# Haian-Jin/TensoIR

Measured on AMD Instinct MI355X. Metric: primary+secondary rays/sec at 4096 rays x 512 samples, higher is better.
Workload: dtype f32 io and field; decoders split-bf16 x3 (hi/lo operands, 3 MFMA products), fp32 accumulate; indirect light (secondary-ray records): fp16 shadow taps + fp16 single-product decoder, fp32 accumulate

## Files before the change

include/tensoir_hip.h:

```cpp
#ifndef TENSOIR_HIP_H
#define TENSOIR_HIP_H

#include <stdint.h>

#ifdef __cplusplus
extern "C" {
#endif

#define TIR_VERSION 100

#define TIR_OK               0
#define TIR_ERR_ARG         -1001
#define TIR_ERR_UNSUPPORTED -1002
#define TIR_ERR_NO_DEVICE   -1003

typedef struct TirField {
    float aabb_min[3];
    float aabb_max[3];
    float inv_aabb[3];
    int32_t grid[3];
    float step_size;
    float distance_scale;
    float density_shift;
    float weight_thres;
// ... 18 lines not shown
    float occ_hi[3];
    int32_t tune_lds_lines;
    int32_t tune_xcd_order;
    const float* dense_sigma;
    int32_t dense_pitch;
} TirField;

typedef struct TirFieldHalf {
    const void* aplane[3];
    const void* aline[3];
} TirFieldHalf;

#define TIR_HALF_MAX_JOBS 8
typedef struct TirHalfJob { const float* src; void* dst; int64_t n; unsigned* absmax; } TirHalfJob;
typedef struct TirHalfJobs { TirHalfJob job[TIR_HALF_MAX_JOBS]; } TirHalfJobs;

typedef struct TirMlp {
    const float* packed;
    int32_t feat_dim;
    int32_t pe;
    int32_t hidden;
    int32_t out_dim;
    int32_t act;
    int32_t tune_grid;
} TirMlp;

typedef struct TirEnvSG {
    const float* sgs;
    const float* rot;
    int32_t n_sg;
    int32_t n_lights;
} TirEnvSG;

int  tir_version(void);
const char* tir_error_string(int code);
int  tir_device_check(void);

int tir_pack_plane(const float* src, float* dst, int32_t C, int32_t H, int32_t W, void* stream);
int tir_pack_occupancy(const float* vol, uint8_t* nbr, int32_t W, int32_t H, int32_t D, void* stream);
int tir_pack_basis(const float* w, float* dst, int32_t app_dim, int32_t n_in, void* stream);
int tir_light_mean(const float* light_line, float* mean, int32_t L, int32_t n, void* stream);
int64_t tir_mlp_packed_floats(int32_t feat_dim, int32_t pe, int32_t hidden, int32_t out_dim);
int tir_pack_mlp(const float* w0, const float* b0, const float* w1, const float* b1,
                 const float* w2, const float* b2, int32_t feat_dim, int32_t pe, int32_t hidden,
                 int32_t out_dim, float* packed, void* stream);

int tir_vm_density_fwd(const TirField* f, const float* xyz, float* feat, float* sigma,
                       int64_t n, void* stream);

int tir_occupancy_query(const TirField* f, const float* xyz, uint8_t* hit, int64_t n, void* stream);

int tir_dense_alpha(const TirField* f, const float* lin_x, const float* lin_y, const float* lin_z,
                    int32_t gx, int32_t gy, int32_t gz, float length, float* alpha, void* stream);
int tir_alpha_pool(const float* alpha, int32_t gx, int32_t gy, int32_t gz, float thres, float* vol,
                   int32_t* bbox, void* stream);
int tir_filter_rays(const TirField* f, const float* rays, int64_t n, int32_t n_samples, int32_t bbox_only,
                    uint8_t* mask, void* stream);

int tir_dense_sigma_build(const TirField* f, float* vol, int32_t pitch, void* stream);
int tir_dense_sigma_fwd(const TirField* f, const float* xyz, float* feat, float* sigma, int64_t n, void* stream);

int tir_density_grad_fwd(const TirField* f, const float* xyz, float* sigma, float* grad,
                         float* normal, int64_t n, const int32_t* n_dev, void* stream);
int tir_density_feat_grad_fwd(const TirField* f, const float* xyz, float* feat, float* grad, int64_t n, void* stream);

int tir_vm_app_fwd(const TirField* f, const float* xyz, const int32_t* light_idx,
                   const int32_t* idx_map, float* rad_feat, float* int_feat, int32_t out_stride,
                   int32_t idx_div, int64_t n, const int32_t* n_dev, void* stream);

int tir_vm_app_jitter_fwd(const TirField* f, const float* xyz, int64_t n, const int32_t* n_dev, float scale,
                          uint64_t seed, uint64_t offset, const int64_t* rng_state, float* xyz_out,
                          float* int_feat, int32_t out_stride, void* stream);

int tir_vm_app_primary_fwd(const TirField* f, const float* xyz, const int32_t* light_idx, const int32_t* idx_map,
                           float* rad_feat, float* int_feat, int32_t out_stride, int64_t n, const int32_t* n_dev,
                           float scale, uint64_t seed, uint64_t offset, const int64_t* rng_state, float* xyz_out,
                           float* int_feat_jit, void* stream);
int tir_vm_app_primary_x3_fwd(const TirField* f, const float* xyz, const int32_t* light_idx, const int32_t* idx_map,
                              float* rad_feat, float* int_feat, int32_t out_stride, int64_t n, const int32_t* n_dev,
                              float scale, uint64_t seed, uint64_t offset, const int64_t* rng_state, float* xyz_out,
                              float* int_feat_jit, void* stream);
int tir_vm_app_fwd_x3(const TirField* f, const float* xyz, const int32_t* light_idx,
                      const int32_t* idx_map, float* rad_feat, float* int_feat, int32_t out_stride,
                      int32_t idx_div, int64_t n, const int32_t* n_dev, void* stream);
int tir_vm_app_fwd_bf16x3(const TirField* f, const float* xyz, const int32_t* light_idx,
                          const int32_t* idx_map, float* rad_feat, float* int_feat, int32_t out_stride,
                          int32_t idx_div, int64_t n, const int32_t* n_dev, void* stream);
int tir_vm_app_fwd_valu(const TirField* f, const float* xyz, const int32_t* light_idx,
                        const int32_t* idx_map, float* rad_feat, float* int_feat, int32_t out_stride,
                        int32_t idx_div, int64_t n, const int32_t* n_dev, void* stream);

int tir_mlp_fwd(const TirMlp* m, const float* feat, int32_t feat_stride, const float* aux,
                const int32_t* aux_map, int32_t aux_mod, float* out, int64_t n, const int32_t* n_dev,
        void* stream);
int tir_mlp_fwd_bf16x3(const TirMlp* m, const float* feat, int32_t feat_stride, const float* aux,
                       const int32_t* aux_map, int32_t aux_mod, float* out, int64_t n, const int32_t* n_dev,
        void* stream);

int tir_pack_half(const float* const* srcs, void* const* dsts, const int64_t* counts, int32_t n_tables, void* stream);
int tir_pack_half_checked(const float* const* srcs, void* const* dsts, const int64_t* counts, int32_t n_tables, float* absmax,
                          void* stream);
int tir_vm_app_fwd_h16(const TirField* f, const TirFieldHalf* fh, const float* xyz, const int32_t* light_idx,
                       const int32_t* idx_map, float* rad_feat, int32_t out_stride, int32_t idx_div, int64_t n,
                       const int32_t* n_dev, void* stream);

int tir_indirect_fused_fwd(const TirField* f, const TirFieldHalf* fh, const TirMlp* m, const float* xyz,
                           const int32_t* light_idx, const int32_t* rec_map, int32_t idx_div, int32_t aux_mod,
                           const float* table, float* out, int64_t n, const int32_t* n_dev, void* stream);

int tir_indirect_fused_hp_fwd(const TirField* f, const TirMlp* m, const float* xyz, const int32_t* light_idx,
                              const int32_t* rec_map, int32_t idx_div, int32_t aux_mod, const float* table, float* out,
                              int64_t n, const int32_t* n_dev, void* stream);

int tir_mlp_fwd_multi_bf16x3(const TirMlp* const* mlps, const float* const* feats, int32_t feat_stride,
                             const float* const* auxs, const int32_t* const* aux_maps, float* const* outs,
                             int32_t n_jobs, int64_t n, const int32_t* n_dev, void* stream);

int tir_mlp_aux_table(const TirMlp* m, const float* aux, int64_t n_aux, float* table, void* stream);
int tir_mlp_fwd_auxtab_bf16x3(const TirMlp* m, const float* feat, int32_t feat_stride, const float* table,
                              const int32_t* aux_map, int32_t aux_mod, float* out, int64_t n, const int32_t* n_dev,
                              void* stream);
int tir_mlp_fwd_auxtab_f16(const TirMlp* m, const float* feat, int32_t feat_stride, const float* table,
                           const int32_t* aux_map, int32_t aux_mod, float* out, int64_t n, const int32_t* n_dev,
                           void* stream);
int tir_mlp_train_fwd_auxtab_bf16x3(const TirMlp* m, const float* feat, int32_t feat_stride, const float* table,
                                    const int32_t* aux_map, int32_t aux_mod, float* out, float* h1, float* h2, int64_t n,
                                    const int32_t* n_dev, void* stream);
int tir_mlp_fwd_multi_auxtab_bf16x3(const TirMlp* const* mlps, const float* const* feats, int32_t feat_stride,
                                    const float* const* auxs, const int32_t* const* aux_maps,
                                    const float* const* tables, float* const* outs, int32_t n_jobs, int64_t n,
                                    const int32_t* n_dev, void* stream);
int tir_mlp_train_fwd_multi_bf16x3(const TirMlp* const* mlps, const float* const* feats, int32_t feat_stride,
                                   const float* const* auxs, const int32_t* const* aux_maps, float* const* outs,
                                   float* const* h1s, float* const* h2s, int32_t n_jobs, int64_t n,
                                   const int32_t* n_dev, void* stream);
int tir_mlp_fwd_bf16(const TirMlp* m, const float* feat, int32_t feat_stride, const float* aux,
                     const int32_t* aux_map, int32_t aux_mod, float* out, int64_t n, const int32_t* n_dev,
        void* stream);
int tir_mlp_fwd_valu(const TirMlp* m, const float* feat, int32_t feat_stride, const float* aux,
                     const int32_t* aux_map, int32_t aux_mod, float* out, int64_t n, const int32_t* n_dev,
        void* stream);

int tir_march_primary_fwd(const TirField* f, const float* rays, const float* ray_jitter,
                          int32_t B, int32_t S, float t_stop, float* weight, float* acc,
                          float* depth, float* t_end, int32_t* app_count,
                          unsigned long long* stats, void* stream);

int tir_march_primary_fused_fwd(const TirField* f, const float* rays, const float* ray_jitter,
                                int32_t B, int32_t S, float t_stop, float* weight, float* acc,
                                float* depth, float* t_end, int32_t* app_count, unsigned long long* stats,
                                float* viewdirs, int32_t* zero_words, int32_t n_zero, int32_t* ticket,
                                int32_t* offsets, int32_t cap, int32_t* total, void* stream);

int tir_exclusive_scan(const int32_t* counts, int32_t* offsets, int32_t n, void* stream);
int tir_exclusive_scan_capped(const int32_t* counts, int32_t* offsets, int32_t n, int32_t cap,
                              int32_t* total, void* stream);

int tir_record_check(const int32_t* const* counters, const int64_t* caps, int32_t n, int64_t* state,
                     int64_t* host_out, void* stream);

int tir_compact_primary(const TirField* f, const float* rays, const float* ray_jitter,
                        const float* weight, const int32_t* offsets, int32_t B, int32_t S,
                        int32_t* rec_ray, int32_t* rec_k, float* rec_w, float* rec_xyz,
                        void* stream);

#define TIR_MAP_STRIDE 20
int tir_composite_primary(const float* rays, const int32_t* offsets, const float* rec_w,
                          const float* rgb, const float* brdf, const float* brdf_jit,
                          const float* pred_normal, const float* derived_normal,
                          const float* acc, const float* depth, int32_t B, int32_t white_bg,
                          int32_t is_relight, float fixed_fresnel, float* out_maps, void* stream);

int tir_composite_primary_fused(const float* rays, const int32_t* offsets, const float* rec_w,
                                const float* rgb, const float* brdf, const float* brdf_jit,
                                const float* pred_normal, const float* derived_normal,
                                const float* acc, const float* depth, int32_t B, int32_t white_bg,
                                int32_t is_relight, float fixed_fresnel, float* out_maps, int32_t* ticket,
                                float* smooth_out, int64_t* rng_state, int64_t rng_step, void* stream);


int tir_march_secondary_fwd(const TirField* f, const float* origins, const int32_t* org_map,
                            const float* dirs, const int32_t* dir_map, const uint8_t* active,
                            int64_t n_rays, int32_t n_dirs, int32_t n_sample, const float* z_vals,
                            float t_stop, float* vis, float* one_minus_acc,
                            int32_t* rec_counter, int64_t rec_cap, int32_t* rec_ray,
                            float* rec_w, float* rec_xyz, int32_t* ray_rec_off,
                            int32_t* ray_rec_cnt, unsigned long long* stats, void* stream);

int tir_march_secondary_ids_fwd(const TirField* f, const float* origins, const int32_t* org_map,
                                const float* dirs, const int32_t* dir_map, const uint8_t* active,
                                int64_t n_rays, int32_t n_dirs, int32_t n_sample, const float* z_vals,
                                float t_stop, float* vis, float* one_minus_acc,
                                int32_t* rec_counter, int64_t rec_cap, int32_t* rec_ray,
                                float* rec_w, float* rec_xyz, int32_t* ray_rec_off,
                                int32_t* ray_rec_cnt, unsigned long long* stats, const int32_t* ray_ids,
                                const int32_t* n_ids_dev, void* stream);

int tir_accumulate_records(const int32_t* ray_rec_off, const int32_t* ray_rec_cnt,
                           const float* rec_w, const float* rec_rgb, int64_t n_rays,
                           float* indirect, void* stream);

int tir_env_sg_fwd(const TirEnvSG* e, const float* dirs, int32_t D, float* out, void* stream);

int tir_env_pixel_fwd(const float* light_rgbs, int32_t H, int32_t W, const float* rot, const float* dirs,
                      int32_t n_lights, int64_t n_dirs, int32_t softplus, float* env, void* stream);
int tir_env_pixel_bwd(const float* light_rgbs, int32_t H, int32_t W, const float* rot, const float* dirs,
                      int32_t n_lights, int64_t n_dirs, const float* g_env, float* g_light, void* stream);

int tir_shade_setup(const float* maps, const float* rays, const float* dirs, int32_t M,
                    int32_t D, float acc_thres, float* surf, uint8_t* active, void* stream);

int tir_shade_setup_compact(const float* maps, const float* rays, const float* dirs, int32_t M,
                            int32_t D, float acc_thres, float* surf, uint8_t* active, int32_t* pair_ids,
                            int32_t* n_active, float* vis, int32_t* ray_rec_cnt, int32_t pair_order, void* stream);

int tir_shade_integrate(const float* maps, const float* rays, const float* dirs,
                        const int32_t* light_idx, const float* vis, const float* indirect,
                        const float* env, const float* weight_d, int32_t M, int32_t D,
                        int32_t n_lights, int32_t equal_area, int32_t use_srgb, float acc_thres,
                        float* out_rgb, void* stream);

int tir_shade_integrate_records(const float* maps, const float* rays, const float* dirs,
                                const int32_t* light_idx, const float* vis, const int32_t* ray_rec_off,
                                const int32_t* ray_rec_cnt, const float* rec_w, const float* rec_rgb,
                                const float* env, const float* weight_d, int32_t M, int32_t D,
                                int32_t n_lights, int32_t equal_area, int32_t use_srgb, float acc_thres,
                                float* out_rgb, int32_t* reset_counter, void* stream);

int tir_relight_importance(const float* normal, const float* albedo, const float* rough,
                           const float* fresnel, const float* rays_d, const float* light_dir,
                           const float* light_rgb, const float* light_pdf, const float* vis,
                           int32_t M, int32_t Ns, float* out_rgb, void* stream);

int tir_env_sample_setup(const float* row_cdf, const float* col_cdf, int32_t H, int32_t W, const float* env_dir,
                         const float* normal, int32_t M, int32_t Ns, uint64_t seed, uint64_t offset,
                         int32_t* cell, uint8_t* active, void* stream);
int tir_env_sample_setup_list(const float* row_cdf, const float* col_cdf, int32_t H, int32_t W, const float* env_dir,
                                int32_t dir_stride, const float* normal, int32_t M, int32_t Ns, uint64_t seed, uint64_t offset,
                                int32_t bins_r, int32_t bins_c, int32_t block_pairs, const int32_t* row_guide,
                                const uint16_t* col_guide, int32_t guide_rows, int32_t guide_cols, int32_t* cell,
                                float* vis, int32_t* pair_ids, int32_t* n_active, void* stream);
int tir_relight_importance_cells(const float* normal, const float* albedo, const float* rough,
                                 const float* fresnel, const float* rays_d, const int32_t* cell,
                                 const float* env_dir, const float* env_rgb, const float* env_pdf,
                                 const float* vis, int32_t M, int32_t Ns, float* out_rgb, void* stream);
int tir_relight_importance_cells_packed(const float* normal, const float* albedo, const float* rough,
                                        const float* fresnel, const float* rays_d, const int32_t* cell,
                                        const float* env_cell, const float* vis, int32_t M, int32_t Ns,
                                        float* out_rgb, void* stream);
int tir_env_lookup(const float* env_rgb, int32_t H, int32_t W, const float* dirs, int64_t n, float* out, void* stream);

int tir_surface_compact(const float* maps, const float* rays, int32_t B, float acc_thres, float* surf, float* normal,
                        float* albedo, float* rough, float* fresnel, float* rays_d, int32_t* slot, int32_t* n_hit,
                        void* stream);
int tir_env_sample_setup_list_n(const float* row_cdf, const float* col_cdf, int32_t H, int32_t W, const float* env_dir,
                                int32_t dir_stride, const float* normal, int32_t M, int32_t Ns, uint64_t seed, uint64_t offset,
                                int32_t bins_r, int32_t bins_c, int32_t block_pairs, const int32_t* row_guide,
                                const uint16_t* col_guide, int32_t guide_rows, int32_t guide_cols, int32_t* cell,
                                float* vis, int32_t* pair_ids, int32_t* n_active, const int32_t* m_dev, void* stream);
int tir_relight_importance_cells_packed_n(const float* normal, const float* albedo, const float* rough,
                                          const float* fresnel, const float* rays_d, const int32_t* cell,
                                          const float* env_cell, const float* vis, int32_t M, int32_t Ns,
                                          float* out_rgb, const int32_t* m_dev, void* stream);
int tir_env_compose(const float* env_rgb, int32_t H, int32_t W, const float* dirs, int32_t dir_stride, int64_t n,
                    const int32_t* slot, const float* fg_rgb, float* out, int32_t out_stride, void* stream);

int tir_ggx_specular(const float* normal, const float* v, const float* l, const float* rough,
                     const float* fresnel, int32_t M, int32_t D, float* spec, void* stream);

typedef struct TirFieldGrad {
    float* dplane[3];
    float* dline[3];
    float* aplane[3];
    float* aline[3];
    float* light_line;
    float* light_mean;
} TirFieldGrad;

int tir_march_primary_train_fwd(const TirField* f, const float* rays, const float* ray_jitter,
                                int32_t B, int32_t S, float t_stop, float* weight, float* sigma,
                                float* acc, float* depth, float* t_end, int32_t* app_count, void* stream);

int tir_composite_primary_bwd(const float* rays, const int32_t* offsets, const int32_t* rec_k,
                              const float* rec_w, const float* rgb, const float* brdf,
                              const float* brdf_jit, const float* pred_normal,
                              const float* derived_normal, const float* acc, const float* depth,
                              int32_t B, int32_t S, int32_t white_bg, int32_t is_relight,
                              float fixed_fresnel, const float* g_maps, float* g_rgb, float* g_brdf,
                              float* g_brdf_jit, float* g_pred, float* g_der, float* g_weight,
                              float* g_acc, float* g_depth, void* stream);

int tir_march_primary_bwd(const TirField* f, const TirFieldGrad* g, const float* rays,
                          const float* ray_jitter, int32_t B, int32_t S, const float* sigma,
                          const float* weight, const float* g_weight, const float* g_acc,
                          const float* g_depth, float* g_feature, void* stream);

int tir_density_grad_bwd(const TirField* f, const TirFieldGrad* g, const float* xyz,
                         const float* g_normal, int64_t n, void* stream);

int tir_vm_density_bwd(const TirField* f, const TirFieldGrad* g, const float* xyz, const float* g_feat, int64_t n,
                       void* stream);
int tir_density_feat_bwd(const TirField* f, const TirFieldGrad* g, const float* xyz, const float* g_feat,
                         float* g_xyz_out, int64_t n, void* stream);
int tir_density_feat_grad_bwd(const TirField* f, const TirFieldGrad* g, const float* xyz, const float* v,
                              float* g_xyz_out, int64_t n, void* stream);

int tir_vm_app_bwd(const TirField* f, const TirFieldGrad* g, const float* xyz,
                   const int32_t* light_idx, const int32_t* idx_map, const float* g_rad,
                   const float* g_int, int32_t stride, int64_t n, float* y_rad, float* y_int,
                   void* stream);

int tir_mlp_train_fwd(const TirMlp* m, const float* feat, int32_t feat_stride, const float* aux,
                      const int32_t* aux_map, int32_t aux_mod, float* out, float* h1, float* h2,
                      int64_t n, const int32_t* n_dev, void* stream);
int tir_mlp_train_fwd_bf16x3(const TirMlp* m, const float* feat, int32_t feat_stride, const float* aux,
                             const int32_t* aux_map, int32_t aux_mod, float* out, float* h1, float* h2,
                             int64_t n, const int32_t* n_dev, void* stream);
int tir_mlp_inputs(const TirMlp* m, const float* feat, int32_t feat_stride, const float* aux,
                   const int32_t* aux_map, int32_t aux_mod, float* x, int64_t n, void* stream);
int64_t tir_mlp_bwd_packed_floats(int32_t feat_dim, int32_t pe, int32_t hidden, int32_t out_dim);
int tir_pack_mlp_bwd(const float* w0, const float* w1, const float* w2, int32_t feat_dim, int32_t pe,
                     int32_t hidden, int32_t out_dim, float* packed, void* stream);
int tir_mlp_bwd(const TirMlp* m, const float* packed_bwd, const float* feat, int32_t feat_stride,
                const float* out, const float* g_out, const float* h1, const float* h2, int64_t n,
                float* g_feat, float* dz1, float* dz2, float* dz3, void* stream);
int tir_mlp_bwd_bf16x3(const TirMlp* m, const float* packed_bwd, const float* feat, int32_t feat_stride,
                const float* out, const float* g_out, const float* h1, const float* h2, int64_t n,
                float* g_feat, float* dz1, float* dz2, float* dz3, void* stream);
int tir_mlp_bwd_multi_bf16x3(const TirMlp* const* mlps, const float* const* packed_bwds, const float* const* feats,
                             int32_t feat_stride, const float* const* outs, const float* const* g_outs,
                             const float* const* h1s, const float* const* h2s, int32_t n_jobs, int64_t n,
                             float* const* g_feats, float* const* dz1s, float* const* dz2s, float* const* dz3s, void* stream);

int tir_gemm_tn_small_bf16x3(const float* const* As, int32_t lda, int32_t M, const float* const* Bs, int32_t ldb,
                             int32_t N, int32_t n_jobs, int64_t n, float* C, int32_t ldc, void* stream);

int tir_mlp_wgrad_multi(const float* const* dz1s, const float* const* dz2s, const float* const* dz3s,
                        const float* const* h1s, const float* const* h2s, const float* const* feats,
                        int32_t feat_stride, const float* const* auxs, const int32_t* const* aux_maps,
                        float* const* dW0s, float* const* db0s, float* const* dW1s, float* const* db1s,
                        float* const* dW2s, float* const* db2s, int32_t n_jobs, int64_t n, int32_t max_workgroups,
                        void* stream);

int tir_gemm_tn(const float* A, int32_t lda, int32_t M, const float* B, int32_t ldb, int32_t N,
                int32_t ones_col, int64_t n, float* C, int32_t ldc, float* bias_out, void* stream);
int tir_gemm_tn_bf16x3(const float* A, int32_t lda, int32_t M, const float* B, int32_t ldb, int32_t N,
                int32_t ones_col, int64_t n, float* C, int32_t ldc, float* bias_out, void* stream);

int tir_adam_step(int32_t n_tensors, float* const* p, const float* const* g, float* const* m, float* const* v,
                  const int64_t* count, const float* lr, const float* bias_correction1,
                  const float* bias_correction2, float beta1, float beta2, float eps, void* stream);

int tir_shade_integrate_bwd(const float* maps, const float* rays, const float* dirs,
                            const int32_t* light_idx, const float* vis, const float* indirect,
                            const float* env, const float* weight_d, int32_t M, int32_t D,
                            int32_t n_lights, int32_t equal_area, int32_t use_srgb, float acc_thres,
                            const float* g_out, float* g_maps, float* g_env, void* stream);

int tir_env_sg_bwd(const TirEnvSG* e, const float* dirs, int32_t D, const float* g_env, float* g_sgs,
                   void* stream);

int64_t tir_mc_blocks(int32_t gx, int32_t gy, int32_t gz);
int tir_mc_count(const float* vol, int32_t gx, int32_t gy, int32_t gz, float level, int32_t* counts, int32_t* offsets,
                 void* stream);
int tir_mc_emit(const float* vol, int32_t gx, int32_t gy, int32_t gz, float level, float spacing_x, float spacing_y,
                float spacing_z, float origin_x, float origin_y, float origin_z, const int32_t* offsets, int32_t n_verts,
                int32_t n_faces, int32_t* vbase, float* verts, float* normals, int32_t* faces, void* stream);
// ... 100 lines not shown
```

tensoir_amd/_lib.py:

```python
from __future__ import annotations

import ctypes as C
import os

_HERE = os.path.dirname(os.path.abspath(__file__))
LIB_PATH = os.environ.get("TENSOIR_HIP_LIB", os.path.join(_HERE, "libtensoir_hip.so"))

c_float_p = C.c_void_p
c_int_p = C.c_void_p


class TirField(C.Structure):
    _fields_ = [
        ("aabb_min", C.c_float * 3), ("aabb_max", C.c_float * 3), ("inv_aabb", C.c_float * 3),
        ("grid", C.c_int32 * 3),
        ("step_size", C.c_float), ("distance_scale", C.c_float), ("density_shift", C.c_float),
        ("weight_thres", C.c_float), ("near_", C.c_float), ("far_", C.c_float),
        ("act", C.c_int32), ("n_dcomp", C.c_int32), ("n_acomp", C.c_int32), ("app_dim", C.c_int32),
        ("n_lights", C.c_int32),
        ("dplane", C.c_void_p * 3), ("dline", C.c_void_p * 3),
        ("aplane", C.c_void_p * 3), ("aline", C.c_void_p * 3),
        ("basis_t", C.c_void_p), ("light_line", C.c_void_p), ("light_mean", C.c_void_p),
        ("occ_nbr", C.c_void_p),
        ("occ_dim", C.c_int32 * 3), ("occ_aabb_min", C.c_float * 3), ("occ_inv", C.c_float * 3),
        ("occ_lo", C.c_float * 3), ("occ_hi", C.c_float * 3),
        ("tune_lds_lines", C.c_int32), ("tune_xcd_order", C.c_int32),
        ("dense_sigma", C.c_void_p), ("dense_pitch", C.c_int32),
    ]


class TirFieldHalf(C.Structure):
    _fields_ = [("aplane", C.c_void_p * 3), ("aline", C.c_void_p * 3)]


class TirFieldGrad(C.Structure):
    _fields_ = [("dplane", C.c_void_p * 3), ("dline", C.c_void_p * 3), ("aplane", C.c_void_p * 3),
                ("aline", C.c_void_p * 3), ("light_line", C.c_void_p), ("light_mean", C.c_void_p)]


class TirMlp(C.Structure):
    _fields_ = [("packed", C.c_void_p), ("feat_dim", C.c_int32), ("pe", C.c_int32),
                ("hidden", C.c_int32), ("out_dim", C.c_int32), ("act", C.c_int32), ("tune_grid", C.c_int32)]


class TirEnvSG(C.Structure):
    _fields_ = [("sgs", C.c_void_p), ("rot", C.c_void_p), ("n_sg", C.c_int32), ("n_lights", C.c_int32)]


P = C.c_void_p
I32 = C.c_int32
I64 = C.c_int64
F32 = C.c_float

SIGNATURES = {
    "tir_version": (C.c_int, []),
    "tir_error_string": (C.c_char_p, [C.c_int]),
    "tir_device_check": (C.c_int, []),
    "tir_pack_plane": (C.c_int, [P, P, I32, I32, I32, P]),
    "tir_pack_occupancy": (C.c_int, [P, P, I32, I32, I32, P]),
    "tir_pack_basis": (C.c_int, [P, P, I32, I32, P]),
    "tir_light_mean": (C.c_int, [P, P, I32, I32, P]),
    "tir_mlp_packed_floats": (I64, [I32, I32, I32, I32]),
    "tir_pack_mlp": (C.c_int, [P, P, P, P, P, P, I32, I32, I32, I32, P, P]),
    "tir_vm_density_fwd": (C.c_int, [C.POINTER(TirField), P, P, P, I64, P]),
    "tir_occupancy_query": (C.c_int, [C.POINTER(TirField), P, P, I64, P]),
    "tir_dense_alpha": (C.c_int, [C.POINTER(TirField), P, P, P, I32, I32, I32, F32, P, P]),
    "tir_alpha_pool": (C.c_int, [P, I32, I32, I32, F32, P, P, P]),
    "tir_filter_rays": (C.c_int, [C.POINTER(TirField), P, I64, I32, I32, P, P]),
    "tir_dense_sigma_build": (C.c_int, [C.POINTER(TirField), P, I32, P]),
    "tir_dense_sigma_fwd": (C.c_int, [C.POINTER(TirField), P, P, P, I64, P]),
    "tir_density_grad_fwd": (C.c_int, [C.POINTER(TirField), P, P, P, P, I64, P, P]),
    "tir_density_feat_grad_fwd": (C.c_int, [C.POINTER(TirField), P, P, P, I64, P]),
    "tir_vm_app_fwd": (C.c_int, [C.POINTER(TirField), P, P, P, P, P, I32, I32, I64, P, P]),
    "tir_vm_app_fwd_bf16x3": (C.c_int, [C.POINTER(TirField), P, P, P, P, P, I32, I32, I64, P, P]),
    "tir_vm_app_fwd_x3": (C.c_int, [C.POINTER(TirField), P, P, P, P, P, I32, I32, I64, P, P]),
    "tir_pack_half": (C.c_int, [P, P, P, I32, P]),
    "tir_pack_half_checked": (C.c_int, [P, P, P, I32, P, P]),
    "tir_vm_app_fwd_h16": (C.c_int, [C.POINTER(TirField), C.POINTER(TirFieldHalf), P, P, P, P, I32, I32, I64, P, P]),
    "tir_indirect_fused_fwd": (C.c_int, [C.POINTER(TirField), C.POINTER(TirFieldHalf), C.POINTER(TirMlp), P, P, P, I32, I32, P, P, I64, P, P]),
    "tir_indirect_fused_hp_fwd": (C.c_int, [C.POINTER(TirField), C.POINTER(TirMlp), P, P, P, I32, I32, P, P, I64, P, P]),
    "tir_vm_app_fwd_valu": (C.c_int, [C.POINTER(TirField), P, P, P, P, P, I32, I32, I64, P, P]),
    "tir_mlp_fwd": (C.c_int, [C.POINTER(TirMlp), P, I32, P, P, I32, P, I64, P, P]),
    "tir_mlp_fwd_bf16x3": (C.c_int, [C.POINTER(TirMlp), P, I32, P, P, I32, P, I64, P, P]),
    "tir_mlp_fwd_multi_bf16x3": (C.c_int, [P, P, I32, P, P, P, I32, I64, P, P]),
    "tir_mlp_fwd_multi_auxtab_bf16x3": (C.c_int, [P, P, I32, P, P, P, P, I32, I64, P, P]),
    "tir_mlp_aux_table": (C.c_int, [C.POINTER(TirMlp), P, I64, P, P]),
    "tir_mlp_fwd_auxtab_bf16x3": (C.c_int, [C.POINTER(TirMlp), P, I32, P, P, I32, P, I64, P, P]),
    "tir_mlp_fwd_auxtab_f16": (C.c_int, [C.POINTER(TirMlp), P, I32, P, P, I32, P, I64, P, P]),
    "tir_mlp_train_fwd_auxtab_bf16x3": (C.c_int, [C.POINTER(TirMlp), P, I32, P, P, I32, P, P, P, I64, P, P]),
    "tir_mlp_train_fwd_multi_bf16x3": (C.c_int, [P, P, I32, P, P, P, P, P, I32, I64, P, P]),
    "tir_mlp_fwd_bf16": (C.c_int, [C.POINTER(TirMlp), P, I32, P, P, I32, P, I64, P, P]),
    "tir_mlp_fwd_valu": (C.c_int, [C.POINTER(TirMlp), P, I32, P, P, I32, P, I64, P, P]),
    "tir_march_primary_fwd": (C.c_int, [C.POINTER(TirField), P, P, I32, I32, F32, P, P, P, P, P, P, P]),
    "tir_exclusive_scan": (C.c_int, [P, P, I32, P]),
    "tir_exclusive_scan_capped": (C.c_int, [P, P, I32, I32, P, P]),
    "tir_march_primary_fused_fwd": (C.c_int, [C.POINTER(TirField), P, P, I32, I32, F32, P, P, P, P, P, P,
                                              P, P, I32, P, P, I32, P, P]),
    "tir_composite_primary_fused": (C.c_int, [P, P, P, P, P, P, P, P, P, P, I32, I32, I32, F32, P, P, P, P, I64, P]),
    "tir_vm_app_jitter_fwd": (C.c_int, [C.POINTER(TirField), P, I64, P, F32, C.c_uint64, C.c_uint64, P, P, P, I32, P]),
    "tir_vm_app_primary_fwd": (C.c_int, [C.POINTER(TirField), P, P, P, P, P, I32, I64, P, F32, C.c_uint64, C.c_uint64, P, P, P, P]),
    "tir_vm_app_primary_x3_fwd": (C.c_int, [C.POINTER(TirField), P, P, P, P, P, I32, I64, P, F32, C.c_uint64, C.c_uint64, P, P, P, P]),
    "tir_compact_primary": (C.c_int, [C.POINTER(TirField), P, P, P, P, I32, I32, P, P, P, P, P]),
    "tir_composite_primary": (C.c_int, [P, P, P, P, P, P, P, P, P, P, I32, I32, I32, F32, P, P]),
    "tir_march_secondary_fwd": (C.c_int, [C.POINTER(TirField), P, P, P, P, P, I64, I32, I32, P, F32, P, P,
                                          P, I64, P, P, P, P, P, P, P]),
    "tir_accumulate_records": (C.c_int, [P, P, P, P, I64, P, P]),
    "tir_env_sg_fwd": (C.c_int, [C.POINTER(TirEnvSG), P, I32, P, P]),
    "tir_env_pixel_fwd": (C.c_int, [P, I32, I32, P, P, I32, I64, I32, P, P]),
    "tir_env_pixel_bwd": (C.c_int, [P, I32, I32, P, P, I32, I64, P, P, P]),
    "tir_shade_setup": (C.c_int, [P, P, P, I32, I32, F32, P, P, P]),
    "tir_shade_integrate": (C.c_int, [P, P, P, P, P, P, P, P, I32, I32, I32, I32, I32, F32, P, P]),
    "tir_shade_integrate_records": (C.c_int, [P, P, P, P, P, P, P, P, P, P, P, I32, I32, I32, I32, I32, F32, P, P, P]),
    "tir_shade_setup_compact": (C.c_int, [P, P, P, I32, I32, F32, P, P, P, P, P, P, I32, P]),
    "tir_march_secondary_ids_fwd": (C.c_int, [C.POINTER(TirField), P, P, P, P, P, I64, I32, I32, P, F32, P, P,
                                              P, I64, P, P, P, P, P, P, P, P, P]),
    "tir_relight_importance": (C.c_int, [P, P, P, P, P, P, P, P, P, I32, I32, P, P]),
    "tir_env_sample_setup": (C.c_int, [P, P, I32, I32, P, P, I32, I32, C.c_uint64, C.c_uint64, P, P, P]),
    "tir_env_sample_setup_list": (C.c_int, [P, P, I32, I32, P, I32, P, I32, I32, C.c_uint64, C.c_uint64, I32, I32, I32, P, P, I32, I32, P, P, P, P, P]),
    "tir_relight_importance_cells": (C.c_int, [P, P, P, P, P, P, P, P, P, P, I32, I32, P, P]),
    "tir_relight_importance_cells_packed": (C.c_int, [P, P, P, P, P, P, P, P, I32, I32, P, P]),
    "tir_env_lookup": (C.c_int, [P, I32, I32, P, I64, P, P]),
    "tir_surface_compact": (C.c_int, [P, P, I32, C.c_float, P, P, P, P, P, P, P, P, P]),
    "tir_env_sample_setup_list_n": (C.c_int, [P, P, I32, I32, P, I32, P, I32, I32, C.c_uint64, C.c_uint64, I32, I32, I32, P, P, I32, I32, P, P, P, P, P, P]),
    "tir_relight_importance_cells_packed_n": (C.c_int, [P, P, P, P, P, P, P, P, I32, I32, P, P, P]),
    "tir_env_compose": (C.c_int, [P, I32, I32, P, I32, I64, P, P, P, I32, P]),
    "tir_ggx_specular": (C.c_int, [P, P, P, P, P, I32, I32, P, P]),
    "tir_march_primary_train_fwd": (C.c_int, [C.POINTER(TirField), P, P, I32, I32, F32, P, P, P, P, P, P, P]),
    "tir_composite_primary_bwd": (C.c_int, [P] * 11 + [I32, I32, I32, I32, F32] + [P] * 9 + [P]),
    "tir_march_primary_bwd": (C.c_int, [C.POINTER(TirField), C.POINTER(TirFieldGrad), P, P, I32, I32, P, P, P, P, P, P, P]),
    "tir_density_grad_bwd": (C.c_int, [C.POINTER(TirField), C.POINTER(TirFieldGrad), P, P, I64, P]),
    "tir_vm_density_bwd": (C.c_int, [C.POINTER(TirField), C.POINTER(TirFieldGrad), P, P, I64, P]),
    "tir_density_feat_bwd": (C.c_int, [C.POINTER(TirField), C.POINTER(TirFieldGrad), P, P, P, I64, P]),
    "tir_density_feat_grad_bwd": (C.c_int, [C.POINTER(TirField), C.POINTER(TirFieldGrad), P, P, P, I64, P]),
    "tir_vm_app_bwd": (C.c_int, [C.POINTER(TirField), C.POINTER(TirFieldGrad), P, P, P, P, P, I32, I64, P, P, P]),
    "tir_mlp_train_fwd": (C.c_int, [C.POINTER(TirMlp), P, I32, P, P, I32, P, P, P, I64, P, P]),
    "tir_mlp_train_fwd_bf16x3": (C.c_int, [C.POINTER(TirMlp), P, I32, P, P, I32, P, P, P, I64, P, P]),
    "tir_mlp_inputs": (C.c_int, [C.POINTER(TirMlp), P, I32, P, P, I32, P, I64, P]),
    "tir_mlp_bwd_packed_floats": (I64, [I32, I32, I32, I32]),
    "tir_pack_mlp_bwd": (C.c_int, [P, P, P, I32, I32, I32, I32, P, P]),
    "tir_mlp_bwd": (C.c_int, [C.POINTER(TirMlp), P, P, I32, P, P, P, P, I64, P, P, P, P, P]),
    "tir_mlp_bwd_bf16x3": (C.c_int, [C.POINTER(TirMlp), P, P, I32, P, P, P, P, I64, P, P, P, P, P]),
    "tir_mlp_bwd_multi_bf16x3": (C.c_int, [P, P, P, I32, P, P, P, P, I32, I64, P, P, P, P, P]),
    "tir_gemm_tn_small_bf16x3": (C.c_int, [P, I32, I32, P, I32, I32, I32, I64, P, I32, P]),
    "tir_mlp_wgrad_multi": (C.c_int, [P, P, P, P, P, P, I32, P, P, P, P, P, P, P, P, I32, I64, I32, P]),
    "tir_record_check": (C.c_int, [P, P, I32, P, P, P]),
    "tir_adam_step": (C.c_int, [I32, P, P, P, P, P, P, P, P, F32, F32, F32, P]),
    "tir_gemm_tn": (C.c_int, [P, I32, I32, P, I32, I32, I32, I64, P, I32, P, P]),
    "tir_gemm_tn_bf16x3": (C.c_int, [P, I32, I32, P, I32, I32, I32, I64, P, I32, P, P]),
    "tir_shade_integrate_bwd": (C.c_int, [P, P, P, P, P, P, P, P, I32, I32, I32, I32, I32, F32, P, P, P, P]),
    "tir_env_sg_bwd": (C.c_int, [C.POINTER(TirEnvSG), P, I32, P, P, P]),
    "tir_mc_blocks": (I64, [I32, I32, I32]),
    "tir_mc_count": (C.c_int, [P, I32, I32, I32, F32, P, P, P]),
    "tir_mc_emit": (C.c_int, [P, I32, I32, I32, F32, F32, F32, F32, F32, F32, F32, P, I32, I32, P, P, P, P, P]),
    "tir_ccl_blocks": (I64, [I32, I32, I32]),
    "tir_ccl_label": (C.c_int, [P, I32, I32, I32, F32, I32, P, P, P, P]),
    "tir_ccl_table": (C.c_int, [P, I32, I32, I32, P, I32, P, P, P, P]),
    "tir_ccl_filter": (C.c_int, [P, P, I32, I32, I32, F32, P, P, I32, F32, P, P]),
    "tir_simplify_blocks": (I64, [I64]),
    "tir_simplify_count": (C.c_int, [P, I64, P, I64, C.POINTER(C.c_float), C.POINTER(C.c_float), C.POINTER(I32), P, P, P, P, P, P]),
    "tir_simplify_emit": (C.c_int, [P, I64, P, I64, C.POINTER(C.c_float), C.POINTER(C.c_float), C.POINTER(I32), C.c_double, P, P,
                                    I32, I32, P, P, P, P, P, P]),
    "tir_bake_composite": (C.c_int, [P, P, P, P, P, P, P, P, P, C.POINTER(C.c_float), I64, I64, P, P]),
    "tir_irradiance_integrate": (C.c_int, [P, P, P, P, P, P, I64, I32, I32, P, P]),
    "tir_atlas_corners": (C.c_int, [P, I64, P, P, I64, I32, I32, I32, P, P, P, P, P, P]),
    "tir_atlas_texels": (C.c_int, [P, I64, P, P, I64, I32, I32, I32, P, P, P, P, P]),
    "tir_atlas_pack": (C.c_int, [P, I64, P, P, I64, I32, I32, I32, P, P, P, P, P, P, P, P, P, P, P]),
    "tir_raster_project": (C.c_int, [P, I64, P, I64, C.POINTER(C.c_float), F32, I32, I32, F32, P, P, P]),
    "tir_raster_cover": (C.c_int, [P, I64, I32, I32, I32, P, P, P]),
    "tir_raster_resolve": (C.c_int, [P, I64, P, I32, I32, P, P]),
    "tir_raster_shade": (C.c_int, [P, I64, P, P, P, P, P, P, I32, I32, I32, I32, P, P]),
    "tir_env_cells": (C.c_int, [P, I32, I32, P, I32, I32, P, P]),
    "tir_light_gbuffer": (C.c_int, [P, P, P, I64, I32, F32, I32, P, P]),
    "tir_shadow_maps": (C.c_int, [P, I64, P, I64, P, I32, I32, P, P, I32, P, P]),
    "tir_shadow_lookup": (C.c_int, [P, P, P, P, P, I64, I32, I32, F32, F32, P, P]),
    "tir_light_gbuffer_shadowed": (C.c_int, [P, P, P, P, P, P, I64, I32, I32, F32, F32, F32, I32, P, P]),
    "tir_ssim_workspace": (I64, [I64, I32, I32, I32, I32]),
    "tir_ssim": (C.c_int, [P, P, I64, I32, I32, I32, P, I32, C.c_double, C.c_double, P, P, P, P]),
    "tir_image_error_workspace": (I64, [I64, I64]),
    "tir_image_error": (C.c_int, [P, P, P, I64, I64, I32, I32, P, P, P]),
    "tir_tv_workspace": (I64, [I32, P, P, P]),
    "tir_tv_fwd": (C.c_int, [P, P, P, P, P, I32, P, P, P, P]),
    "tir_tv_bwd": (C.c_int, [P, P, P, P, P, I32, P, P, P]),
}

_lib = None


class TensoirHipError(RuntimeError):
    pass


def lib():
    global _lib
    if _lib is not None:
        return _lib
    if not os.path.exists(LIB_PATH):
        raise TensoirHipError(
            f"{LIB_PATH} not found: the HIP library is not built.  Run "
            "`python -c 'import __graft_entry__ as g; g.build()'` (or tensoir_amd/csrc/build.sh). "
            "tensoir_amd has no CPU / eager fallback by design.")
    handle = C.CDLL(LIB_PATH)
    for name, (res, args) in SIGNATURES.items():
        fn = getattr(handle, name)
        fn.restype = res
        fn.argtypes = args
    _lib = handle
    return _lib


def check(rc, what=""):
    if rc != 0:
        msg = lib().tir_error_string(int(rc))
        raise TensoirHipError(f"{what or 'libtensoir_hip'} failed: rc={rc} ({msg.decode() if msg else '?'})")
```

tensoir_amd/csrc/tir_common.hpp:

```cpp
#pragma once
#include <hip/hip_runtime.h>
#include <stdint.h>
#include <initializer_list>
#include <type_traits>
#include "tensoir_hip.h"

#define TIR_WAVE 64

#define TIR_CHECK_LAUNCH()                                   \
    do {                                                     \
        hipError_t e__ = hipGetLastError();                  \
        if (e__ != hipSuccess) return -(int)e__;             \
    } while (0)

static inline hipStream_t tir_stream(void* s) { return reinterpret_cast<hipStream_t>(s); }

static inline int tir_xcd_mapping(const TirField* f) { return f->tune_xcd_order == 1 ? 1 : 0; }

#include <mutex>
#include <set>
#include <utility>
static inline int tir_allow_dynamic_lds(const void* kernel, int bytes) {
    static std::mutex mu;
    static std::set<std::pair<const void*, int>> done;
// ... 677 lines not shown
    t0 -= 1e-4f; t1 += 1e-4f;
}

struct UDiv { unsigned d, m; };
__device__ __forceinline__ UDiv make_udiv(int d) { return UDiv{d > 1 ? (unsigned)d : 1u, d > 1 ? 0xFFFFFFFFu / (unsigned)d : 0u}; }
__device__ __forceinline__ unsigned udiv(unsigned x, const UDiv& u, unsigned& rem) {
    if (u.d == 1) { rem = 0; return x; }
    unsigned q = __umulhi(x, u.m), r = x - q * u.d;
    if (r >= u.d) { q += 1; r -= u.d; }
    rem = r;
    return q;
}

__device__ __forceinline__ float linear2srgb(float x) {
    x = fminf(fmaxf(x, 0.0f), 1.0f);
    float lin = x * 12.92f;
    float nonlin = 1.055f * powf(x + 1e-6f, 0.41666666666666667f) - 0.055f;
    return (x <= 0.0031308f) ? lin : nonlin;
}

struct RaySetup {
    float o[3], d[3];
    float t_min;
};

__device__ __forceinline__ RaySetup ray_setup(const TirField& f, const float* __restrict__ rays, int r) {
    RaySetup s;
    float tm = -INFINITY;
#pragma unroll
    for (int a = 0; a < 3; ++a) {
        s.o[a] = rays[6 * (size_t)r + a];
        s.d[a] = rays[6 * (size_t)r + 3 + a];
        float vec = (s.d[a] == 0.0f) ? 1e-6f : s.d[a];
        float ra = __fdiv_rn(sub_rn(f.aabb_max[a], s.o[a]), vec);
        float rb = __fdiv_rn(sub_rn(f.aabb_min[a], s.o[a]), vec);
        tm = fmaxf(tm, fminf(ra, rb));
    }
    s.t_min = fminf(fmaxf(tm, f.near_), f.far_);
    return s;
}

__device__ __forceinline__ float sample_z(const TirField& f, float t_min, int k, float jitter, bool has_jitter) {
    float rng = (float)k;
    if (has_jitter) rng = add_rn(rng, jitter);
    return add_rn(t_min, mul_rn(f.step_size, rng));
}



__device__ __forceinline__ void philox_round(uint32_t (&c)[4], uint32_t k0, uint32_t k1) {
    const uint64_t p0 = (uint64_t)0xD2511F53u * c[0], p1 = (uint64_t)0xCD9E8D57u * c[2];
    const uint32_t n0 = (uint32_t)(p1 >> 32) ^ c[1] ^ k0, n2 = (uint32_t)(p0 >> 32) ^ c[3] ^ k1;
    c[0] = n0; c[1] = (uint32_t)p1; c[2] = n2; c[3] = (uint32_t)p0;
}

__device__ __forceinline__ void jitter_normals(unsigned long long seed, unsigned long long offset, uint64_t idx, float (&nrm)[3]) {
    uint32_t c[4] = {(uint32_t)idx, (uint32_t)(idx >> 32), (uint32_t)offset, (uint32_t)(offset >> 32)};
    uint32_t k0 = (uint32_t)seed, k1 = (uint32_t)(seed >> 32);
#pragma unroll
    for (int r = 0; r < 10; ++r) { philox_round(c, k0, k1); k0 += 0x9E3779B9u; k1 += 0xBB67AE85u; }
    const float u0 = ((float)c[0] + 0.5f) * 2.3283064365386963e-10f, u1 = ((float)c[1] + 0.5f) * 2.3283064365386963e-10f;
    const float u2 = ((float)c[2] + 0.5f) * 2.3283064365386963e-10f, u3 = ((float)c[3] + 0.5f) * 2.3283064365386963e-10f;
    const float r0 = sqrtf(-2.0f * logf(fminf(u0, 0.99999994f))), r1 = sqrtf(-2.0f * logf(fminf(u2, 0.99999994f)));
    float s0, c0, s1, c1;
    sincospif(2.0f * u1, &s0, &c0);
    sincospif(2.0f * u3, &s1, &c1);
    nrm[0] = r0 * c0; nrm[1] = r0 * s0; nrm[2] = r1 * c1;
    (void)s1;
}

__device__ __forceinline__ void philox_uniform4(unsigned long long seed, unsigned long long offset, uint64_t idx, float (&u)[4]) {
    uint32_t c[4] = {(uint32_t)idx, (uint32_t)(idx >> 32), (uint32_t)offset, (uint32_t)(offset >> 32)};
    uint32_t k0 = (uint32_t)seed, k1 = (uint32_t)(seed >> 32);
#pragma unroll
    for (int r = 0; r < 10; ++r) { philox_round(c, k0, k1); k0 += 0x9E3779B9u; k1 += 0xBB67AE85u; }
#pragma unroll
    for (int q = 0; q < 4; ++q) u[q] = fminf(((float)c[q] + 0.5f) * 2.3283064365386963e-10f, 0.99999994f);
}

struct XcdRange { long long first, end, stride; };
__device__ __forceinline__ XcdRange xcd_range_at(long long n_items, int per, bool on, int bid, int nblk) {
    XcdRange r;
    if (!on || (nblk & 7) != 0) {
        r.first = (long long)bid * per; r.end = n_items; r.stride = (long long)nblk * per;
        return r;
    }
    const int xcd = bid & 7, local = bid >> 3, per_xcd = nblk >> 3;
    const long long chunk = (n_items + 7) / 8;
    const long long lo = chunk * xcd;
    r.first = lo + (long long)local * per;
    r.end = lo + chunk < n_items ? lo + chunk : n_items;
    r.stride = (long long)per_xcd * per;
    return r;
}
__device__ __forceinline__ XcdRange xcd_range(long long n_items, int per, bool on) {
    return xcd_range_at(n_items, per, on, (int)blockIdx.x, (int)gridDim.x);
}

template <int G>
__device__ __forceinline__ void record_sum(const float* __restrict__ rec_w, const float* __restrict__ rec_rgb, int b, int e,
                                           float (&acc)[3]) {
    int i = b;
    for (; e - i >= G; i += G) {
        float w[G], c[G][3];
#pragma unroll
        for (int j = 0; j < G; ++j) {
            w[j] = rec_w[i + j];
            c[j][0] = rec_rgb[3 * (size_t)(i + j)]; c[j][1] = rec_rgb[3 * (size_t)(i + j) + 1]; c[j][2] = rec_rgb[3 * (size_t)(i + j) + 2];
        }
#pragma unroll
        for (int j = 0; j < G; ++j) {
            acc[0] = fmaf(w[j], c[j][0], acc[0]); acc[1] = fmaf(w[j], c[j][1], acc[1]); acc[2] = fmaf(w[j], c[j][2], acc[2]);
        }
    }
    if (i < e) {
        float w[G - 1], c[G - 1][3];
#pragma unroll
        for (int j = 0; j < G - 1; ++j) {
            const size_t k = (size_t)min(i + j, e - 1);
            w[j] = rec_w[k];
            c[j][0] = rec_rgb[3 * k]; c[j][1] = rec_rgb[3 * k + 1]; c[j][2] = rec_rgb[3 * k + 2];
        }
#pragma unroll
        for (int j = 0; j < G - 1; ++j)
            if (i + j < e) {
                acc[0] = fmaf(w[j], c[j][0], acc[0]); acc[1] = fmaf(w[j], c[j][1], acc[1]); acc[2] = fmaf(w[j], c[j][2], acc[2]);
            }
    }
}
constexpr int RECORD_GROUP = 8;

#define TIR_TAIL_THREADS 256

__device__ __forceinline__ double block_sum(double v, double* s4) {
#pragma unroll
    for (int d = 32; d > 0; d >>= 1) v += __shfl_xor(v, d, 64);
    __syncthreads();
    if ((threadIdx.x & 63) == 0) s4[threadIdx.x >> 6] = v;
    __syncthreads();
    return (s4[0] + s4[1]) + (s4[2] + s4[3]);
}

__device__ __forceinline__ bool last_of_image(int32_t* ticket, int per_image, int* s_last) {
    if (threadIdx.x == 0) {
        asm volatile("s_waitcnt vmcnt(0)" ::: "memory");
        const int t = __hip_atomic_fetch_add(ticket, 1, __ATOMIC_RELAXED, __HIP_MEMORY_SCOPE_AGENT);
        *s_last = (t == per_image - 1);
        if (*s_last) __hip_atomic_store(ticket, 0, __ATOMIC_RELAXED, __HIP_MEMORY_SCOPE_AGENT);
    }
    __syncthreads();
    return *s_last != 0;
}

}
```

tensoir_amd/csrc/tir_march.hip:

```cpp
#include "tir_common.hpp"

using namespace tir;

__device__ __forceinline__ void march_one_ray(const TirField& f, const float* __restrict__ rays, const float* __restrict__ ray_jitter,
                                              int B, int S, float t_stop, float* __restrict__ weight, float* __restrict__ acc_out,
                                              float* __restrict__ depth_out, float* __restrict__ tend_out,
                                              int32_t* __restrict__ app_count, unsigned long long* __restrict__ stats,
                                              float* __restrict__ sigma_out, float* __restrict__ viewdirs, bool coh, int ray, int lane) {
    RaySetup rs = ray_setup(f, rays, ray);
    if (viewdirs && lane < 3) viewdirs[3 * (size_t)ray + lane] = rays[6 * (size_t)ray + 3 + lane];

    const bool hj = ray_jitter != nullptr;
    const float jit = hj ? ray_jitter[ray] : 0.0f;

    __shared__ __attribute__((aligned(16))) float wl_all[4][256];
    float* wl = wl_all[threadIdx.x >> 6];
    float T = 1.0f;
    float acc = 0.0f, depth = 0.0f;
    int cnt = 0;
    int k0 = 0;
    unsigned n_gather = 0;
    for (; k0 < S; k0 += 64) {
        const int k = k0 + lane;
        float z = 0.0f, x = 0.f, y = 0.f, zz = 0.f;
        bool valid = false;
        if (k < S) {
            z = sample_z(f, rs.t_min, k, jit, hj);
            float px = add_rn(rs.o[0], mul_rn(rs.d[0], z));
            float py = add_rn(rs.o[1], mul_rn(rs.d[1], z));
            float pz = add_rn(rs.o[2], mul_rn(rs.d[2], z));
            valid = sample_valid(f, px, py, pz, x, y, zz);
        }
        const float sigma = wave_sigma(f, valid, x, y, zz, wl);
        float w = 0.0f, v = 1.0f;
        if (k < S) {
            float dist = (k + 1 < S) ? sub_rn(sample_z(f, rs.t_min, k + 1, jit, hj), z) : 0.0f;
            float alpha = 1.0f - expf(-sigma * mul_rn(dist, f.distance_scale));
            v = add_rn(sub_rn(1.0f, alpha), 1e-10f);
            w = alpha;
        }
        float incl = scan_prod<64>(v, lane);
        float excl = shift_up1<64>(incl, lane);
        w = w * (T * excl);
        if (k < S) weight[(size_t)ray * S + k] = w;
        if (sigma_out && k < S) sigma_out[(size_t)ray * S + k] = sigma;
        acc += w;
        depth = fmaf(w, z, depth);
        cnt += __popcll(__ballot(w > f.weight_thres));
        if (stats) n_gather += __popcll(__ballot(valid));
        T = T * __shfl(incl, 63, 64);
        if (T < t_stop) { k0 += 64; break; }
    }
    for (; k0 < S; k0 += 64) {
        const int k = k0 + lane;
        if (k < S) weight[(size_t)ray * S + k] = 0.0f;
        if (sigma_out && k < S) sigma_out[(size_t)ray * S + k] = 0.0f;
    }
    acc = group_sum<64>(acc);
    depth = group_sum<64>(depth);
    if (lane == 0) {
        acc_out[ray] = acc;
        depth_out[ray] = depth;
        if (tend_out) tend_out[ray] = T;
        if (coh) __hip_atomic_store(app_count + ray, cnt, __ATOMIC_RELAXED, __HIP_MEMORY_SCOPE_AGENT);
        else app_count[ray] = cnt;
        if (stats) atomicAdd(stats, (unsigned long long)n_gather);
    }
}


struct TirMarchExtras {
    float* viewdirs;
    int32_t* zero_words; int n_zero;
    int32_t* ticket; int32_t* offsets; int cap; int32_t* total_out;
};

__device__ __forceinline__ void block_exclusive_scan_capped(const int32_t* __restrict__ counts, int32_t* __restrict__ offsets,
                                                             int n, int cap, int32_t* __restrict__ total_out) {
    constexpr int SCAN_PER = 16;
    __shared__ int32_t wsum[4];
    __shared__ int32_t carry_s;
    const int tid = threadIdx.x, lane = tid & 63, wv = tid >> 6;
    if (tid == 0) carry_s = 0;
    __syncthreads();
    for (int base = 0; base < n; base += 256 * SCAN_PER) {
        const int i0 = base + SCAN_PER * tid;
        int32_t v[SCAN_PER];
#pragma unroll
        for (int j = 0; j < SCAN_PER; ++j)
            v[j] = __hip_atomic_load(counts + min(i0 + j, n - 1), __ATOMIC_RELAXED, __HIP_MEMORY_SCOPE_AGENT);
        int32_t sum = 0;
#pragma unroll
        for (int j = 0; j < SCAN_PER; ++j) {
            const int32_t x = (i0 + j < n) ? v[j] : 0;
            v[j] = sum;
            sum += x;
        }
        int32_t incl = sum;
#pragma unroll
        for (int d = 1; d < 64; d <<= 1) {
            int32_t o = __shfl_up(incl, d, 64);
            if (lane >= d) incl += o;
        }
        if (lane == 63) wsum[wv] = incl;
        __syncthreads();
        int32_t woff = 0;
        for (int q = 0; q < wv; ++q) woff += wsum[q];
        const int32_t carry = carry_s;
        const int32_t first = carry + woff + incl - sum;
#pragma unroll
        for (int j = 0; j < SCAN_PER; ++j)
            if (i0 + j < n) offsets[i0 + j] = min(first + v[j], cap);
        __syncthreads();
        if (tid == 255) carry_s = carry + woff + incl;
        __syncthreads();
    }
    if (tid == 0) {
        offsets[n] = min(carry_s, cap);
        if (total_out) *total_out = carry_s;
    }
}

__global__ void __launch_bounds__(256)
k_march_primary(TirField f, const float* __restrict__ rays, const float* __restrict__ ray_jitter,
                int B, int S, float t_stop, float* __restrict__ weight, float* __restrict__ acc_out,
                float* __restrict__ depth_out, float* __restrict__ tend_out, int32_t* __restrict__ app_count,
                unsigned long long* __restrict__ stats, float* __restrict__ sigma_out, TirMarchExtras ex) {
    const int lane = threadIdx.x & 63;
    const int ray = blockIdx.x * (blockDim.x >> 6) + (threadIdx.x >> 6);
    if (ex.zero_words && blockIdx.x == 0 && threadIdx.x < ex.n_zero) ex.zero_words[threadIdx.x] = 0;
    if (ray < B) march_one_ray(f, rays, ray_jitter, B, S, t_stop, weight, acc_out, depth_out, tend_out, app_count, stats,
                               sigma_out, ex.viewdirs, ex.ticket != nullptr, ray, lane);
    if (!ex.ticket) return;
    __shared__ int s_last;
    asm volatile("s_waitcnt vmcnt(0)" ::: "memory");
    __syncthreads();
    if (threadIdx.x == 0) {
        const int t = __hip_atomic_fetch_add(ex.ticket, 1, __ATOMIC_RELAXED, __HIP_MEMORY_SCOPE_AGENT);
        s_last = (t == (int)gridDim.x - 1);
        if (s_last) __hip_atomic_store(ex.ticket, 0, __ATOMIC_RELAXED, __HIP_MEMORY_SCOPE_AGENT);
    }
    __syncthreads();
    if (s_last) block_exclusive_scan_capped(app_count, ex.offsets, B, ex.cap, ex.total_out);
}

extern "C" int tir_march_primary_fwd(const TirField* f, const float* rays, const float* ray_jitter,
                                     int32_t B, int32_t S, float t_stop, float* weight, float* acc,
                                     float* depth, float* t_end, int32_t* app_count,
                                     unsigned long long* stats, void* stream) {
    if (!f || B < 0 || S <= 0) return TIR_ERR_ARG;
    if (B == 0) return TIR_OK;
    if (!rays || !weight || !acc || !depth || !app_count) return TIR_ERR_ARG;
    if (!(f->n_dcomp == 4 || f->n_dcomp == 8 || f->n_dcomp == 16 || f->n_dcomp == 32)) return TIR_ERR_UNSUPPORTED;
    if (!tir_occ_index_ok(f) || !tir_plane_index_ok(f)) return TIR_ERR_UNSUPPORTED;
    hipLaunchKernelGGL(k_march_primary, dim3((B + 3) / 4), dim3(256), 0, tir_stream(stream), *f, rays,
                       ray_jitter, B, S, t_stop, weight, acc, depth, t_end, app_count, stats, (float*)nullptr, TirMarchExtras{});
    TIR_CHECK_LAUNCH();
    return TIR_OK;
}

extern "C" int tir_march_primary_fused_fwd(const TirField* f, const float* rays, const float* ray_jitter,
                                           int32_t B, int32_t S, float t_stop, float* weight, float* acc,
                                           float* depth, float* t_end, int32_t* app_count, unsigned long long* stats,
                                           float* viewdirs, int32_t* zero_words, int32_t n_zero, int32_t* ticket,
                                           int32_t* offsets, int32_t cap, int32_t* total, void* stream) {
    if (!f || B < 0 || S <= 0 || n_zero < 0 || n_zero > 256 || cap < 0) return TIR_ERR_ARG;
    if ((ticket == nullptr) != (offsets == nullptr)) return TIR_ERR_ARG;
    if (B == 0) return TIR_OK;
    if (!rays || !weight || !acc || !depth || !app_count) return TIR_ERR_ARG;
    if (!(f->n_dcomp == 4 || f->n_dcomp == 8 || f->n_dcomp == 16 || f->n_dcomp == 32)) return TIR_ERR_UNSUPPORTED;
    if (!tir_occ_index_ok(f) || !tir_plane_index_ok(f)) return TIR_ERR_UNSUPPORTED;
    TirMarchExtras ex{viewdirs, zero_words, n_zero, ticket, offsets, cap, total};
    hipLaunchKernelGGL(k_march_primary, dim3((B + 3) / 4), dim3(256), 0, tir_stream(stream), *f, rays,
                       ray_jitter, B, S, t_stop, weight, acc, depth, t_end, app_count, stats, (float*)nullptr, ex);
    TIR_CHECK_LAUNCH();
    return TIR_OK;
}

extern "C" int tir_march_primary_train_fwd(const TirField* f, const float* rays, const float* ray_jitter,
                                           int32_t B, int32_t S, float t_stop, float* weight, float* sigma,
                                           float* acc, float* depth, float* t_end, int32_t* app_count, void* stream) {
    if (!f || B < 0 || S <= 0) return TIR_ERR_ARG;
    if (B == 0) return TIR_OK;
    if (!rays || !weight || !sigma || !acc || !depth || !app_count) return TIR_ERR_ARG;
    if (!(f->n_dcomp == 4 || f->n_dcomp == 8 || f->n_dcomp == 16 || f->n_dcomp == 32)) return TIR_ERR_UNSUPPORTED;
    if (!tir_occ_index_ok(f) || !tir_plane_index_ok(f)) return TIR_ERR_UNSUPPORTED;
    hipLaunchKernelGGL(k_march_primary, dim3((B + 3) / 4), dim3(256), 0, tir_stream(stream), *f, rays,
                       ray_jitter, B, S, t_stop, weight, acc, depth, t_end, app_count,
                       (unsigned long long*)nullptr, sigma, TirMarchExtras{});
    TIR_CHECK_LAUNCH();
    return TIR_OK;
}

__global__ void __launch_bounds__(1024)
k_exclusive_scan(const int32_t* __restrict__ counts, int32_t* __restrict__ offsets, int n, int cap,
                 int32_t* __restrict__ total_out) {
    __shared__ int32_t wsum[16];
    __shared__ int32_t carry_s;
    const int tid = threadIdx.x, lane = tid & 63, wv = tid >> 6;
    if (tid == 0) carry_s = 0;
    __syncthreads();
    for (int base = 0; base < n; base += 1024) {
        int i = base + tid;
        int32_t v = (i < n) ? counts[i] : 0;
        int32_t incl = v;
#pragma unroll
        for (int d = 1; d < 64; d <<= 1) {
            int32_t o = __shfl_up(incl, d, 64);
            if (lane >= d) incl += o;
        }
        if (lane == 63) wsum[wv] = incl;
        __syncthreads();
        int32_t woff = 0;
        for (int q = 0; q < wv; ++q) woff += wsum[q];
        int32_t carry = carry_s;
        if (i < n) offsets[i] = min(carry + woff + incl - v, cap);
        __syncthreads();
        if (tid == 1023) carry_s = carry + woff + incl;
        __syncthreads();
    }
    if (tid == 0) {
        offsets[n] = min(carry_s, cap);
        if (total_out) *total_out = carry_s;
    }
}

extern "C" int tir_exclusive_scan(const int32_t* counts, int32_t* offsets, int32_t n, void* stream) {
    if (!offsets || n < 0 || (n > 0 && !counts)) return TIR_ERR_ARG;
    hipLaunchKernelGGL(k_exclusive_scan, dim3(1), dim3(1024), 0, tir_stream(stream), counts, offsets, n, 0x7fffffff,
                       (int32_t*)nullptr);
    TIR_CHECK_LAUNCH();
    return TIR_OK;
}

extern "C" int tir_exclusive_scan_capped(const int32_t* counts, int32_t* offsets, int32_t n, int32_t cap,
                                         int32_t* total, void* stream) {
    if (!offsets || n < 0 || cap < 0 || (n > 0 && !counts)) return TIR_ERR_ARG;
    hipLaunchKernelGGL(k_exclusive_scan, dim3(1), dim3(1024), 0, tir_stream(stream), counts, offsets, n, cap, total);
    TIR_CHECK_LAUNCH();
    return TIR_OK;
}

struct TirCheck4 { const int32_t* cnt[4]; int64_t cap[4]; int n; };

__global__ void k_record_check(TirCheck4 c, int64_t* __restrict__ state, int64_t* __restrict__ host_out) {
    if (threadIdx.x != 0 || blockIdx.x != 0) return;
    int64_t over = state[4];
    for (int i = 0; i < 4; ++i) {
        int64_t v = 0;
        if (i < c.n) {
            v = *c.cnt[i];
            if (v > c.cap[i]) over = 1;
            if (v > state[i]) state[i] = v;
        }
        host_out[i] = v;
        host_out[4 + i] = state[i];
    }
    state[4] = over;
    host_out[8] = over;
    __threadfence_system();
}

extern "C" int tir_record_check(const int32_t* const* counters, const int64_t* caps, int32_t n, int64_t* state,
                                int64_t* host_out, void* stream) {
    if (n < 0 || n > 4 || !state || !host_out || (n > 0 && (!counters || !caps))) return TIR_ERR_ARG;
    TirCheck4 c;
    c.n = n;
    for (int i = 0; i < 4; ++i) { c.cnt[i] = i < n ? counters[i] : nullptr; c.cap[i] = i < n ? caps[i] : 0; }
    for (int i = 0; i < n; ++i) if (!c.cnt[i]) return TIR_ERR_ARG;
    hipLaunchKernelGGL(k_record_check, dim3(1), dim3(64), 0, tir_stream(stream), c, state, host_out);
    TIR_CHECK_LAUNCH();
    return TIR_OK;
}

__global__ void __launch_bounds__(256)
k_compact_primary(TirField f, const float* __restrict__ rays, const float* __restrict__ ray_jitter,
                  const float* __restrict__ weight, const int32_t* __restrict__ offsets, int B, int S,
                  int32_t* __restrict__ rec_ray, int32_t* __restrict__ rec_k, float* __restrict__ rec_w,
                  float* __restrict__ rec_xyz) {
    const int lane = threadIdx.x & 63;
    const int ray = blockIdx.x * (blockDim.x >> 6) + (threadIdx.x >> 6);
    if (ray >= B) return;
    int base = offsets[ray];
    const int end = offsets[ray + 1];
    if (end == base) return;
    RaySetup rs = ray_setup(f, rays, ray);
    const bool hj = ray_jitter != nullptr;
    const float jit = hj ? ray_jitter[ray] : 0.0f;
    for (int k0 = 0; k0 < S; k0 += 64) {
        const int k = k0 + lane;
        float w = (k < S) ? weight[(size_t)ray * S + k] : 0.0f;
        bool keep = w > f.weight_thres;
        unsigned long long m = __ballot(keep);
        const int slot = base + __popcll(m & ((1ull << lane) - 1ull));
        if (keep && slot < end) {
            float z = sample_z(f, rs.t_min, k, jit, hj);
            rec_ray[slot] = ray;
            rec_k[slot] = k;
            rec_w[slot] = w;
#pragma unroll
            for (int a = 0; a < 3; ++a) {
                float p = add_rn(rs.o[a], mul_rn(rs.d[a], z));
                rec_xyz[3 * (size_t)slot + a] = norm_coord(p, f.aabb_min[a], f.inv_aabb[a]);
            }
        }
        base += __popcll(m);
    }
}

extern "C" int tir_compact_primary(const TirField* f, const float* rays, const float* ray_jitter,
                                   const float* weight, const int32_t* offsets, int32_t B, int32_t S,
                                   int32_t* rec_ray, int32_t* rec_k, float* rec_w, float* rec_xyz,
                                   void* stream) {
    if (!f || B < 0 || S <= 0) return TIR_ERR_ARG;
    if (B == 0) return TIR_OK;
    if (!rays || !weight || !offsets || !rec_ray || !rec_k || !rec_w || !rec_xyz) return TIR_ERR_ARG;
    hipLaunchKernelGGL(k_compact_primary, dim3((B + 3) / 4), dim3(256), 0, tir_stream(stream), *f, rays,
                       ray_jitter, weight, offsets, B, S, rec_ray, rec_k, rec_w, rec_xyz);
    TIR_CHECK_LAUNCH();
    return TIR_OK;
}

struct TirCompositeExtras {
    int32_t* ticket; float* smooth_out;
    long long* rng_bump; long long rng_step;
};

__device__ __forceinline__ void composite_one_ray(const float* __restrict__ rays, const int32_t* __restrict__ offsets,
                    const float* __restrict__ rec_w, const float* __restrict__ rgb,
                    const float* __restrict__ brdf, const float* __restrict__ brdf_jit,
                    const float* __restrict__ pred_n, const float* __restrict__ der_n,
                    const float* __restrict__ acc_in, const float* __restrict__ depth_in, int white_bg,
                    int is_relight, float fixed_fresnel, float* __restrict__ out, bool coh, int r, int lane) {
    const int b = offsets[r], e = offsets[r + 1];
    float c[3] = {0, 0, 0}, nm[3] = {0, 0, 0}, al[3] = {0, 0, 0};
    float rough = 0, ndiff = 0, norient = 0, albc = 0, rghc = 0;
    const float vd[3] = {rays[6 * (size_t)r + 3], rays[6 * (size_t)r + 4], rays[6 * (size_t)r + 5]};
    for (int i = b + lane; i < e; i += 64) {
        const float w = rec_w[i];
        if (rgb) { c[0] = fmaf(w, rgb[3 * (size_t)i], c[0]); c[1] = fmaf(w, rgb[3 * (size_t)i + 1], c[1]); c[2] = fmaf(w, rgb[3 * (size_t)i + 2], c[2]); }
        if (!is_relight) continue;
        float a3[3] = {0, 0, 0}, rg = 0;
        if (brdf) {
            const float4 bv = *reinterpret_cast<const float4*>(brdf + 4 * (size_t)i);
            a3[0] = bv.x; a3[1] = bv.y; a3[2] = bv.z;
            rg = bv.w * 0.9f + 0.09f;
            al[0] = fmaf(w, a3[0], al[0]); al[1] = fmaf(w, a3[1], al[1]); al[2] = fmaf(w, a3[2], al[2]);
            rough = fmaf(w, rg, rough);
        }
        if (brdf && brdf_jit) {
            const float4 jv = *reinterpret_cast<const float4*>(brdf_jit + 4 * (size_t)i);
            const float ajv[3] = {jv.x, jv.y, jv.z};
            float cost = 0.f;
#pragma unroll
            for (int q = 0; q < 3; ++q) {
                float base = fmaxf(fmaxf(a3[q], ajv[q]), 1e-6f);
                float dlt = (a3[q] - ajv[q]) / base;
                cost = fmaf(dlt, dlt, cost);
            }
            albc = fmaf(w, cost, albc);
            float rj = jv.w * 0.9f + 0.09f;
            float base = fmaxf(fmaxf(rg, rj), 1e-6f);
            float dlt = (rg - rj) / base;
            rghc = fmaf(w, dlt * dlt, rghc);
        }
        if (pred_n) {
            float p3[3] = {pred_n[3 * (size_t)i], pred_n[3 * (size_t)i + 1], pred_n[3 * (size_t)i + 2]};
            nm[0] = fmaf(w, p3[0], nm[0]); nm[1] = fmaf(w, p3[1], nm[1]); nm[2] = fmaf(w, p3[2], nm[2]);
            if (der_n) {
                float d0 = p3[0] - der_n[3 * (size_t)i], d1 = p3[1] - der_n[3 * (size_t)i + 1], d2 = p3[2] - der_n[3 * (size_t)i + 2];
                ndiff = fmaf(w, d0 * d0 + d1 * d1 + d2 * d2, ndiff);
            }
            float dot = vd[0] * p3[0] + vd[1] * p3[1] + vd[2] * p3[2];
            norient = fmaf(w, fmaxf(dot, 0.f), norient);
        }
    }
#pragma unroll
    for (int q = 0; q < 3; ++q) { c[q] = group_sum<64>(c[q]); }
    if (is_relight) {
#pragma unroll
        for (int q = 0; q < 3; ++q) { nm[q] = group_sum<64>(nm[q]); al[q] = group_sum<64>(al[q]); }
        rough = group_sum<64>(rough); ndiff = group_sum<64>(ndiff); norient = group_sum<64>(norient);
        albc = group_sum<64>(albc); rghc = group_sum<64>(rghc);
    }
    if (lane != 0) return;
    const float acc = acc_in[r];
    float depth = depth_in[r];
    float* o = out + (size_t)r * TIR_MAP_STRIDE;
    const float bg = 1.0f - acc;
    if (!is_relight) {
        if (white_bg) { depth = depth + bg * rays[6 * (size_t)r + 5]; c[0] += bg; c[1] += bg; c[2] += bg; }
        o[0] = c[0]; o[1] = c[1]; o[2] = c[2]; o[3] = depth;
        for (int q = 4; q < TIR_MAP_STRIDE; ++q) o[q] = 0.f;
        o[14] = acc;
        return;
    }
    float fr = fixed_fresnel;
    if (white_bg) {
        depth = depth + bg * rays[6 * (size_t)r + 5];
        c[0] += bg; c[1] += bg; c[2] += bg;
        nm[2] += bg;
        al[0] += bg; al[1] += bg; al[2] += bg;
        rough += bg;
        fr += bg;
    }
    o[0] = linear2srgb(c[0]); o[1] = linear2srgb(c[1]); o[2] = linear2srgb(c[2]);
    o[3] = depth;
    float nn = fmaxf(sqrtf(nm[0] * nm[0] + nm[1] * nm[1] + nm[2] * nm[2]), 1e-6f);
    o[4] = nm[0] / nn; o[5] = nm[1] / nn; o[6] = nm[2] / nn;
    o[7] = fminf(fmaxf(al[0], 0.f), 1.f); o[8] = fminf(fmaxf(al[1], 0.f), 1.f); o[9] = fminf(fmaxf(al[2], 0.f), 1.f);
    o[10] = fminf(fmaxf(rough, 0.f), 1.f);
    fr = fminf(fmaxf(fr, 0.f), 1.f);
    o[11] = fr; o[12] = fr; o[13] = fr;
    o[14] = acc;
    o[15] = ndiff; o[16] = norient; o[19] = 0.f;
    if (coh) {
        __hip_atomic_store(o + 17, albc, __ATOMIC_RELAXED, __HIP_MEMORY_SCOPE_AGENT);
        __hip_atomic_store(o + 18, rghc, __ATOMIC_RELAXED, __HIP_MEMORY_SCOPE_AGENT);
    } else { o[17] = albc; o[18] = rghc; }
}


__global__ void __launch_bounds__(256)
k_composite_primary(const float* __restrict__ rays, const int32_t* __restrict__ offsets,
                    const float* __restrict__ rec_w, const float* __restrict__ rgb,
                    const float* __restrict__ brdf, const float* __restrict__ brdf_jit,
                    const float* __restrict__ pred_n, const float* __restrict__ der_n,
                    const float* __restrict__ acc_in, const float* __restrict__ depth_in, int B, int white_bg,
                    int is_relight, float fixed_fresnel, float* __restrict__ out, TirCompositeExtras ex) {
    const int lane = threadIdx.x & 63;
    const int r = blockIdx.x * (blockDim.x >> 6) + (threadIdx.x >> 6);
    if (ex.rng_bump && blockIdx.x == 0 && threadIdx.x == 0) ex.rng_bump[1] += ex.rng_step;
    if (r < B) composite_one_ray(rays, offsets, rec_w, rgb, brdf, brdf_jit, pred_n, der_n, acc_in, depth_in, white_bg,
                                 is_relight, fixed_fresnel, out, ex.ticket != nullptr, r, lane);
    if (!ex.ticket || !is_relight) return;
    __shared__ int s_last;
    __shared__ float s_part[2][4];
    asm volatile("s_waitcnt vmcnt(0)" ::: "memory");
    __syncthreads();
    if (threadIdx.x == 0) {
        const int t = __hip_atomic_fetch_add(ex.ticket, 1, __ATOMIC_RELAXED, __HIP_MEMORY_SCOPE_AGENT);
        s_last = (t == (int)gridDim.x - 1);
        if (s_last) __hip_atomic_store(ex.ticket, 0, __ATOMIC_RELAXED, __HIP_MEMORY_SCOPE_AGENT);
    }
    __syncthreads();
    if (!s_last) return;
    float a = 0.0f, g = 0.0f;
    for (int i = threadIdx.x; i < B; i += 256) {
        a += __hip_atomic_load(out + (size_t)i * TIR_MAP_STRIDE + 17, __ATOMIC_RELAXED, __HIP_MEMORY_SCOPE_AGENT);
        g += __hip_atomic_load(out + (size_t)i * TIR_MAP_STRIDE + 18, __ATOMIC_RELAXED, __HIP_MEMORY_SCOPE_AGENT);
    }
    a = group_sum<64>(a); g = group_sum<64>(g);
    if (lane == 0) { s_part[0][threadIdx.x >> 6] = a; s_part[1][threadIdx.x >> 6] = g; }
    __syncthreads();
    if (threadIdx.x == 0) {
        ex.smooth_out[0] = ((s_part[0][0] + s_part[0][1]) + (s_part[0][2] + s_part[0][3])) / (float)B;
        ex.smooth_out[1] = ((s_part[1][0] + s_part[1][1]) + (s_part[1][2] + s_part[1][3])) / (float)B;
    }
}

extern "C" int tir_composite_primary(const float* rays, const int32_t* offsets, const float* rec_w,
                                     const float* rgb, const float* brdf, const float* brdf_jit,
                                     const float* pred_normal, const float* derived_normal,
                                     const float* acc, const float* depth, int32_t B, int32_t white_bg,
                                     int32_t is_relight, float fixed_fresnel, float* out_maps, void* stream) {
    if (B < 0) return TIR_ERR_ARG;
    if (B == 0) return TIR_OK;
    if (!rays || !offsets || !acc || !depth || !out_maps) return TIR_ERR_ARG;
    hipLaunchKernelGGL(k_composite_primary, dim3((B + 3) / 4), dim3(256), 0, tir_stream(stream), rays, offsets,
                       rec_w, rgb, brdf, brdf_jit, pred_normal, derived_normal, acc, depth, B, white_bg,
                       is_relight, fixed_fresnel, out_maps, TirCompositeExtras{});
    TIR_CHECK_LAUNCH();
    return TIR_OK;
}

extern "C" int tir_composite_primary_fused(const float* rays, const int32_t* offsets, const float* rec_w,
                                           const float* rgb, const float* brdf, const float* brdf_jit,
                                           const float* pred_normal, const float* derived_normal,
                                           const float* acc, const float* depth, int32_t B, int32_t white_bg,
                                           int32_t is_relight, float fixed_fresnel, float* out_maps, int32_t* ticket,
                                           float* smooth_out, int64_t* rng_state, int64_t rng_step, void* stream) {
    if (B < 0 || (ticket == nullptr) != (smooth_out == nullptr)) return TIR_ERR_ARG;
    if (B == 0) return TIR_OK;
    if (!rays || !offsets || !acc || !depth || !out_maps) return TIR_ERR_ARG;
    TirCompositeExtras ex{ticket, smooth_out, reinterpret_cast<long long*>(rng_state), (long long)rng_step};
    hipLaunchKernelGGL(k_composite_primary, dim3((B + 3) / 4), dim3(256), 0, tir_stream(stream), rays, offsets,
                       rec_w, rgb, brdf, brdf_jit, pred_normal, derived_normal, acc, depth, B, white_bg,
                       is_relight, fixed_fresnel, out_maps, ex);
    TIR_CHECK_LAUNCH();
    return TIR_OK;
}

#define TIR_SEC_MAX_SAMPLES 256
#define TIR_SEC_RPB 32

__global__ void __launch_bounds__(256)
k_march_secondary(TirField f, const float* __restrict__ origins, const int32_t* __restrict__ org_map,
                  const float* __restrict__ dirs, const int32_t* __restrict__ dir_map,
                  const uint8_t* __restrict__ active, int64_t n_rays, int n_dirs, int n_sample,
                  const float* __restrict__ z_vals, float t_stop, float* __restrict__ vis,
                  float* __restrict__ one_minus_acc, int32_t* __restrict__ rec_counter, int64_t rec_cap,
                  int32_t* __restrict__ rec_ray, float* __restrict__ rec_w, float* __restrict__ rec_xyz,
                  int32_t* __restrict__ ray_rec_off, int32_t* __restrict__ ray_rec_cnt,
                  unsigned long long* __restrict__ stats, int xcd_on, const int32_t* __restrict__ ray_ids,
                  const int32_t* __restrict__ n_ids_dev) {
    extern __shared__ __attribute__((aligned(16))) float w_lds[];
    int64_t bid = blockIdx.x;
    if (xcd_on && (gridDim.x & 7) == 0) bid = (int64_t)(blockIdx.x & 7) * (gridDim.x >> 3) + (blockIdx.x >> 3);
    if (ray_ids && n_ids_dev) n_rays = min(n_rays, (int64_t)max(*n_ids_dev, 0));
    if (bid * TIR_SEC_RPB >= n_rays) return;
    const int hl = threadIdx.x & 31;
    const int hw = threadIdx.x >> 5;
    const int nz = (n_sample + 3) & ~3;
    float* zt = w_lds;
    float* ws = w_lds + nz + (threadIdx.x >> 6) * 256;
    int* s_cnt = reinterpret_cast<int*>(w_lds + nz + 4 * 256);
    int* s_kstop = s_cnt + TIR_SEC_RPB;
    int* s_base = s_kstop + TIR_SEC_RPB;
    int* s_pid = s_base + TIR_SEC_RPB;
    float* w_all = w_lds + nz + 4 * 256 + 4 * TIR_SEC_RPB;
    for (int i = threadIdx.x; i < n_sample; i += blockDim.x) zt[i] = z_vals[i];
    __syncthreads();
    const bool want_rec = rec_counter != nullptr;
    unsigned n_gather = 0;

    for (int g = 0; g < TIR_SEC_RPB / 8; ++g) {
        const int rl = g * 8 + hw;
        const int64_t slot_id = bid * TIR_SEC_RPB + rl;
        const bool in_range = slot_id < n_rays;
        const int64_t ray = in_range ? (ray_ids ? (int64_t)ray_ids[slot_id] : slot_id) : 0;
        const bool live = in_range && !(active && !active[ray]);
        int cnt = 0, k_stop = n_sample;
        if (__any(live)) {
            float o[3] = {0.f, 0.f, 0.f}, d[3] = {0.f, 0.f, 0.f};
            if (live) {
                const size_t oi = org_map ? (size_t)org_map[ray] : (n_dirs > 0 ? (size_t)((unsigned)ray / (unsigned)n_dirs) : (size_t)ray);
                const size_t di = dir_map ? (size_t)dir_map[ray] : (n_dirs > 0 ? (size_t)((unsigned)ray % (unsigned)n_dirs) : (size_t)ray);
#pragma unroll
                for (int a = 0; a < 3; ++a) { o[a] = origins[3 * oi + a]; d[a] = dirs[3 * di + a]; }
            }
            float* wl = w_all + (size_t)rl * n_sample;
            float T = 1.0f, acc = 0.0f;
            bool done = !live;
            for (int k0 = 0; k0 < n_sample; k0 += 32) {
                const int k = k0 + hl;
                float z = 0.f, x = 0.f, y = 0.f, zz = 0.f;
                bool valid = false;
                const bool on = !done && k < n_sample;
                if (on) {
                    z = zt[k];
                    float px = add_rn(o[0], mul_rn(d[0], z));
                    float py = add_rn(o[1], mul_rn(d[1], z));
                    float pz = add_rn(o[2], mul_rn(d[2], z));
                    valid = sample_valid(f, px, py, pz, x, y, zz);
                }
                const float sigma = wave_sigma(f, valid, x, y, zz, ws);
                float w = 0.0f, v = 1.0f;
                if (on) {
                    float dist = (k + 1 < n_sample) ? sub_rn(zt[k + 1], z) : 0.0f;
                    float alpha = 1.0f - exp_neg_fast(sigma * mul_rn(dist, f.distance_scale));
                    v = add_rn(sub_rn(1.0f, alpha), 1e-10f);
                    w = alpha;
                }
                float incl = scan_prod<32>(v, hl);
                float excl = shift_up1<32>(incl, hl);
                w = w * (T * excl);
                if (want_rec && on) wl[k] = w;
                acc += w;
                const unsigned long long m = __ballot(w > f.weight_thres);
                cnt += __popc((unsigned)(m >> ((threadIdx.x & 32) ? 32 : 0)));
                if (stats) n_gather += __popc((unsigned)(__ballot(valid) >> ((threadIdx.x & 32) ? 32 : 0)));
                T = T * __shfl(incl, 31, 32);
                if (!done && T < t_stop) { done = true; k_stop = min(k0 + 32, n_sample); }
                if (__all(done)) break;
            }
            acc = group_sum<32>(acc);
            if (live && hl == 0) {
                if (vis) vis[ray] = T;
                if (one_minus_acc) one_minus_acc[ray] = 1.0f - acc;
            }
        }
        if (hl == 0) {
            if (in_range && !live) {
                if (vis) vis[ray] = 0.0f;
                if (one_minus_acc) one_minus_acc[ray] = 0.0f;
            }
            s_cnt[rl] = live ? cnt : 0;
            s_kstop[rl] = k_stop;
            s_pid[rl] = in_range ? (int)ray : -1;
        }
    }
    if (stats && hl == 0 && n_gather) atomicAdd(stats, (unsigned long long)n_gather);
    if (!want_rec) return;
    __syncthreads();
    if (threadIdx.x < 32) {
        const int c = s_cnt[hl];
        int incl = c;
#pragma unroll
        for (int dd = 1; dd < 32; dd <<= 1) {
            int oth = __shfl_up(incl, dd, 32);
            if (hl >= dd) incl += oth;
        }
        const int total = __shfl(incl, 31, 32);
        int base = 0;
        if (hl == 31 && total > 0) base = atomicAdd(rec_counter, total);
        base = __shfl(base, 31, 32);
        const bool fits = (int64_t)base + total <= rec_cap;
        if (hl == 31 && total > 0 && fits) atomicMax(rec_counter + 1, base + total);
        const int pid = s_pid[hl];
        if (pid >= 0) {
            ray_rec_off[pid] = base + incl - c;
            ray_rec_cnt[pid] = fits ? c : 0;
        }
        s_base[hl] = (fits && c > 0) ? base + incl - c : -1;
    }
    __syncthreads();
    for (int g = 0; g < TIR_SEC_RPB / 8; ++g) {
        const int rl = g * 8 + hw;
        int base = s_base[rl];
        if (base < 0) continue;
        const int64_t ray = s_pid[rl];
        const size_t oi = org_map ? (size_t)org_map[ray] : (n_dirs > 0 ? (size_t)((unsigned)ray / (unsigned)n_dirs) : (size_t)ray);
        const size_t di = dir_map ? (size_t)dir_map[ray] : (n_dirs > 0 ? (size_t)((unsigned)ray % (unsigned)n_dirs) : (size_t)ray);
        float o[3], d[3];
#pragma unroll
        for (int a = 0; a < 3; ++a) { o[a] = origins[3 * oi + a]; d[a] = dirs[3 * di + a]; }
        const float* wl = w_all + (size_t)rl * n_sample;
        const int k_end = s_kstop[rl];
        const unsigned half_shift = (threadIdx.x & 32) ? 32 : 0;
        for (int q0 = 0; q0 < k_end; q0 += 32) {
            const int k = q0 + hl;
            float w = (k < k_end) ? wl[k] : 0.0f;
            const bool keep = w > f.weight_thres;
            const unsigned hm = (unsigned)(__ballot(keep) >> half_shift);
            if (keep) {
                const int slot = base + __popc(hm & ((1u << hl) - 1u));
                const float z = zt[k];
                rec_ray[slot] = (int32_t)ray;
                rec_w[slot] = w;
#pragma unroll
                for (int a = 0; a < 3; ++a) {
                    float p = add_rn(o[a], mul_rn(d[a], z));
                    rec_xyz[3 * (size_t)slot + a] = norm_coord(p, f.aabb_min[a], f.inv_aabb[a]);
// ... 374 lines not shown
```

tensoir_amd/csrc/tir_shade.hip:

```cpp
#include "tir_common.hpp"

using namespace tir;

namespace {

__device__ __forceinline__ void normalize3(float& x, float& y, float& z, float eps) {
    float n = fmaxf(sqrtf(x * x + y * y + z * z), eps);
    x /= n; y /= n; z /= n;
}

struct Surface {
    float N[3], V[3];
    float NoV;
    float alpha2[3], k[3];
    float fres[3];
    float alb_pi[3];
};

__device__ __forceinline__ Surface make_surface(const float* normal, const float* view, const float* rough3,
                                                const float* fres3, const float* albedo) {
    Surface s;
    s.N[0] = normal[0]; s.N[1] = normal[1]; s.N[2] = normal[2];
    s.V[0] = view[0]; s.V[1] = view[1]; s.V[2] = view[2];
    normalize3(s.V[0], s.V[1], s.V[2], 1e-12f);
    normalize3(s.N[0], s.N[1], s.N[2], 1e-12f);
    float nov = s.V[0] * s.N[0] + s.V[1] * s.N[1] + s.V[2] * s.N[2];
    float sg = (nov > 0.f) ? 1.f : ((nov < 0.f) ? -1.f : 0.f);
    s.N[0] *= sg; s.N[1] *= sg; s.N[2] *= sg;
    nov = s.N[0] * s.V[0] + s.N[1] * s.V[1] + s.N[2] * s.V[2];
    s.NoV = fminf(fmaxf(nov, 1e-6f), 1.f);
#pragma unroll
    for (int c = 0; c < 3; ++c) {
        float r = rough3[c];
        float a = r * r;
        s.alpha2[c] = a * a;
        s.k[c] = (a + 2.f * r + 1.0f) / 8.0f;
        s.fres[c] = fres3[c];
        s.alb_pi[c] = albedo ? albedo[c] / 3.14159265358979323846f : 0.f;
    }
    return s;
}

__device__ __forceinline__ void ggx_dir(const Surface& s, float lx, float ly, float lz, float spec[3]) {
    normalize3(lx, ly, lz, 1e-12f);
    float hx = (lx + s.V[0]) / 2.0f, hy = (ly + s.V[1]) / 2.0f, hz = (lz + s.V[2]) / 2.0f;
    normalize3(hx, hy, hz, 1e-12f);
    float NoL = fminf(fmaxf(s.N[0] * lx + s.N[1] * ly + s.N[2] * lz, 1e-6f), 1.f);
    float NoH = fminf(fmaxf(s.N[0] * hx + s.N[1] * hy + s.N[2] * hz, 1e-6f), 1.f);
    float VoH = fminf(fmaxf(s.V[0] * hx + s.V[1] * hy + s.V[2] * hz, 1e-6f), 1.f);
    float FMi = ((-5.55473f) * VoH - 6.98316f) * VoH;
    float p2 = exp2f(FMi);
    const float four_pi = 4.0f * 3.14159265358979323846f;
#pragma unroll
    for (int c = 0; c < 3; ++c) {
        float frac0 = s.fres[c] + (1.f - s.fres[c]) * p2;
        float frac = frac0 * s.alpha2[c];
        float nom0 = NoH * NoH * (s.alpha2[c] - 1.f) + 1.f;
        float nom1 = s.NoV * (1.f - s.k[c]) + s.k[c];
        float nom2 = NoL * (1.f - s.k[c]) + s.k[c];
        float nom = fminf(fmaxf(four_pi * nom0 * nom0 * nom1 * nom2, 1e-6f), four_pi);
        spec[c] = frac / nom;
    }
}

__global__ void __launch_bounds__(128)
k_env_sg(TirEnvSG e, const float* __restrict__ dirs, int D, float* __restrict__ out) {
    const int ld = blockIdx.x;
    const int l = ld / D, d = ld % D;
    const float v0 = dirs[3 * d], v1 = dirs[3 * d + 1], v2 = dirs[3 * d + 2];
    const float* R = e.rot + 9 * l;
    const float r0 = v0 * R[0] + v1 * R[3] + v2 * R[6];
    const float r1 = v0 * R[1] + v1 * R[4] + v2 * R[7];
    const float r2 = v0 * R[2] + v1 * R[5] + v2 * R[8];
    float c0 = 0.f, c1 = 0.f, c2 = 0.f;
    for (int k = threadIdx.x; k < e.n_sg; k += blockDim.x) {
        const float* g = e.sgs + 7 * k;
        float nrm = sqrtf(g[0] * g[0] + g[1] * g[1] + g[2] * g[2]);
        float dot = r0 * (g[0] / nrm) + r1 * (g[1] / nrm) + r2 * (g[2] / nrm);
        float ex = expf(fabsf(g[3]) * (dot - 1.0f));
        c0 += fabsf(g[4]) * ex; c1 += fabsf(g[5]) * ex; c2 += fabsf(g[6]) * ex;
    }
    __shared__ float red[3][2];
    c0 = group_sum<64>(c0); c1 = group_sum<64>(c1); c2 = group_sum<64>(c2);
    const int wv = threadIdx.x >> 6;
    if ((threadIdx.x & 63) == 0) { red[0][wv] = c0; red[1][wv] = c1; red[2][wv] = c2; }
    __syncthreads();
    if (threadIdx.x == 0) {
        float* o = out + 3 * (size_t)ld;
        o[0] = red[0][0] + red[0][1]; o[1] = red[1][0] + red[1][1]; o[2] = red[2][0] + red[2][1];
    }
}

__global__ void __launch_bounds__(1024)
k_shade_setup(const float* __restrict__ maps, const float* __restrict__ rays, const float* __restrict__ dirs,
              int M, int D, float acc_thres, float* __restrict__ surf, uint8_t* __restrict__ active,
              int32_t* __restrict__ pair_ids, int32_t* __restrict__ n_active, float* __restrict__ vis,
              int32_t* __restrict__ rec_cnt, int dir_major) {
    const int64_t t = (int64_t)blockIdx.x * blockDim.x + threadIdx.x;
    const bool in = t < (int64_t)M * D;
    int64_t i = t;
    if (dir_major && in) i = (t % M) * D + t / M;
    bool act = false;
    if (in) {
        const int m = (int)(i / D), d = (int)(i % D);
        const float* mp = maps + (size_t)m * TIR_MAP_STRIDE;
        const float* r = rays + 6 * (size_t)m;
        if (d == 0) {
            const float depth = mp[3];
#pragma unroll
            for (int a = 0; a < 3; ++a) surf[3 * (size_t)m + a] = add_rn(r[a], mul_rn(depth, r[3 + a]));
        }
        float cs = dirs[3 * d] * mp[4] + dirs[3 * d + 1] * mp[5] + dirs[3 * d + 2] * mp[6];
        act = fmaxf(cs, 0.f) > 1e-6f && mp[14] > acc_thres;
        active[i] = act ? 1 : 0;
    }
    if (!pair_ids) return;
    __shared__ int s_wcnt[16];
    __shared__ int s_base;
    const unsigned long long mask = __ballot(act);
    const int lane = threadIdx.x & 63, wv = threadIdx.x >> 6, nw = blockDim.x >> 6;
    if (lane == 0) s_wcnt[wv] = __popcll(mask);
    __syncthreads();
    if (threadIdx.x == 0) {
        int tot = 0;
        for (int q = 0; q < nw; ++q) { const int c = s_wcnt[q]; s_wcnt[q] = tot; tot += c; }
        s_base = tot ? atomicAdd(n_active, tot) : 0;
    }
    __syncthreads();
    const int base = s_base + s_wcnt[wv];
    if (act) {
        const int64_t slot = (int64_t)base + __popcll(mask & ((1ull << lane) - 1ull));
        if (slot < (int64_t)M * D) pair_ids[slot] = (int32_t)i;
    } else if (in) {
        if (vis) vis[i] = 0.0f;
        if (rec_cnt) rec_cnt[i] = 0;
    }
}

__global__ void __launch_bounds__(256, 4)
k_shade_integrate(const float* __restrict__ maps, const float* __restrict__ rays, const float* __restrict__ dirs,
                  const int32_t* __restrict__ light_idx, const float* __restrict__ vis,
                  const float* __restrict__ indirect, const float* __restrict__ env,
                  const float* __restrict__ weight_d, int M, int D, int n_lights, int equal_area, int use_srgb,
                  float acc_thres, float* __restrict__ out, const int32_t* __restrict__ rec_off,
                  const int32_t* __restrict__ rec_cnt, const float* __restrict__ rec_w, const float* __restrict__ rec_rgb,
                  int32_t* __restrict__ reset_counter) {
    const int lane = threadIdx.x & 63;
    if (reset_counter && blockIdx.x == 0 && threadIdx.x == 0) *reset_counter = 0;
    const int m = blockIdx.x * (blockDim.x >> 6) + (threadIdx.x >> 6);
    if (m >= M) return;
    const float* mp = maps + (size_t)m * TIR_MAP_STRIDE;
    if (!(mp[14] > acc_thres)) {
        if (lane < 3) out[3 * (size_t)m + lane] = 1.0f;
        return;
    }
    const float* r = rays + 6 * (size_t)m;
    float view[3] = {-r[3], -r[4], -r[5]};
    normalize3(view[0], view[1], view[2], 1e-6f);
    const float rough3[3] = {mp[10], mp[10], mp[10]};
    Surface s = make_surface(mp + 4, view, rough3, mp + 11, mp + 7);
    int li = light_idx ? light_idx[m] : 0;
    li = min(max(li, 0), n_lights - 1);
    const float* envl = env + (size_t)li * D * 3;
    float c[3] = {0.f, 0.f, 0.f};
    const bool from_records = !indirect && rec_off;
    for (int d0 = lane; d0 < D; d0 += 128) {
        const bool two = d0 + 64 < D;
        float l2[2][3], e2[2][3], w2[2], v2[2];
        int b2[2] = {0, 0}, n2[2] = {0, 0};
#pragma unroll
        for (int u = 0; u < 2; ++u) {
            const int d = (u && two) ? d0 + 64 : d0;
            const size_t md = (size_t)m * D + d;
#pragma unroll
            for (int q = 0; q < 3; ++q) { l2[u][q] = dirs[3 * d + q]; e2[u][q] = envl[3 * d + q]; }
            w2[u] = equal_area ? 1.0f : weight_d[d];
            v2[u] = vis[md];
            if (from_records) { b2[u] = rec_off[md]; n2[u] = rec_cnt[md]; }
        }
#pragma unroll
        for (int u = 0; u < 2; ++u) {
            if (u && !two) break;
            const float lx = l2[u][0], ly = l2[u][1], lz = l2[u][2];
            const float cosine = fmaxf(lx * mp[4] + ly * mp[5] + lz * mp[6], 0.f);
            float spec[3];
            ggx_dir(s, lx, ly, lz, spec);
            const size_t md = (size_t)m * D + d0 + 64 * u;
            const float v = v2[u];
            const float wd = w2[u];
            float ind[3] = {0.f, 0.f, 0.f};
            if (indirect) { ind[0] = indirect[3 * md]; ind[1] = indirect[3 * md + 1]; ind[2] = indirect[3 * md + 2]; }
            else if (rec_off) record_sum<RECORD_GROUP>(rec_w, rec_rgb, b2[u], b2[u] + n2[u], ind);
#pragma unroll
            for (int q = 0; q < 3; ++q) {
                float light = v * e2[u][q] + ind[q];
                float brdf = s.alb_pi[q] + spec[q];
                if (equal_area) c[q] += 4.0f * 3.14159265358979323846f * brdf * light * cosine;
                else c[q] += brdf * light * cosine * wd;
            }
        }
    }
#pragma unroll
    for (int q = 0; q < 3; ++q) {
        float t = group_sum<64>(c[q]);
        if (equal_area) t /= (float)D;
        t = fminf(fmaxf(t, 0.f), 1.f);
        if (use_srgb) t = linear2srgb(t);
        if (lane == 0) out[3 * (size_t)m + q] = t;
    }
}

__global__ void __launch_bounds__(256)
k_relight_importance(const float* __restrict__ normal, const float* __restrict__ albedo,
                     const float* __restrict__ rough, const float* __restrict__ fresnel,
                     const float* __restrict__ rays_d, const float* __restrict__ ldir,
                     const float* __restrict__ lrgb, const float* __restrict__ lpdf,
                     const float* __restrict__ vis, int M, int Ns, float* __restrict__ out) {
    const int lane = threadIdx.x & 63;
    const int m = blockIdx.x * (blockDim.x >> 6) + (threadIdx.x >> 6);
    if (m >= M) return;
    float view[3] = {-rays_d[3 * (size_t)m], -rays_d[3 * (size_t)m + 1], -rays_d[3 * (size_t)m + 2]};
    normalize3(view[0], view[1], view[2], 1e-6f);
    const float rough3[3] = {rough[m], rough[m], rough[m]};
    const float* nm = normal + 3 * (size_t)m;
    Surface s = make_surface(nm, view, rough3, fresnel + 3 * (size_t)m, albedo + 3 * (size_t)m);
    float c[3] = {0.f, 0.f, 0.f};
    for (int j = lane; j < Ns; j += 64) {
        const size_t mj = (size_t)m * Ns + j;
        const float lx = ldir[3 * mj], ly = ldir[3 * mj + 1], lz = ldir[3 * mj + 2];
        const float cosine = lx * nm[0] + ly * nm[1] + lz * nm[2];
        float spec[3];
        ggx_dir(s, lx, ly, lz, spec);
        const float v = vis[mj], pdf = lpdf[mj];
#pragma unroll
        for (int q = 0; q < 3; ++q)
            c[q] += (s.alb_pi[q] + spec[q]) * (v * lrgb[3 * mj + q]) * cosine / pdf;
    }
#pragma unroll
    for (int q = 0; q < 3; ++q) {
        float t = group_sum<64>(c[q]) / (float)Ns;
        t = linear2srgb(fminf(fmaxf(t, 0.f), 1.f));
        if (lane == 0) out[3 * (size_t)m + q] = t;
    }
}

__device__ __forceinline__ int cdf_upper_bound(const float* __restrict__ cdf, int n, float u) {
    int lo = 0, hi = n - 1;
    while (lo < hi) {
        const int mid = (lo + hi) >> 1;
        if (cdf[mid] > u) hi = mid; else lo = mid + 1;
    }
    return lo;
}

template <typename G>
__device__ __forceinline__ int cdf_upper_bound_guided(const float* __restrict__ cdf, int n, float u, const G* __restrict__ guide, int g) {
    const int k = min((int)(u * (float)g), g - 1);
    int lo = (int)guide[k], hi = (int)guide[k + 1];
    while (lo < hi) {
        const int mid = (lo + hi) >> 1;
        if (cdf[mid] > u) hi = mid; else lo = mid + 1;
    }
    return lo;
}

__global__ void __launch_bounds__(256)
k_env_sample_setup(const float* __restrict__ row_cdf, const float* __restrict__ col_cdf, int H, int W,
                   const float* __restrict__ env_dir, const float* __restrict__ normal, int M, int Ns,
                   unsigned long long seed, unsigned long long offset, int32_t* __restrict__ cell,
                   uint8_t* __restrict__ active) {
    const int64_t i = (int64_t)blockIdx.x * blockDim.x + threadIdx.x;
    if (i >= (int64_t)M * Ns) return;
    const int m = (int)(i / Ns);
    float u[4];
    tir::philox_uniform4(seed, offset, (uint64_t)i, u);
    const int row = cdf_upper_bound(row_cdf, H, u[0]);
    const int col = cdf_upper_bound(col_cdf + (size_t)row * W, W, u[1]);
    const int c = row * W + col;
    cell[i] = c;
    const float* d = env_dir + 3 * (size_t)c;
    const float* nm = normal + 3 * (size_t)m;
    const float cosine = d[0] * nm[0] + d[1] * nm[1] + d[2] * nm[2];
    active[i] = cosine > 1e-6f ? 1 : 0;
}

__global__ void __launch_bounds__(256)
k_env_sample_list(const float* __restrict__ row_cdf, const float* __restrict__ col_cdf, int H, int W,
                    const float* __restrict__ env_dir, int dir_stride, const float* __restrict__ normal, int M, int Ns,
// ... 283 lines not shown
        const float* p = hdr + 3 * ((size_t)i * W + (size_t)b * c);
        for (int j = 0; j < b; ++j) {
            rgb[0] = fmaf(wi, p[3 * j], rgb[0]); rgb[1] = fmaf(wi, p[3 * j + 1], rgb[1]); rgb[2] = fmaf(wi, p[3 * j + 2], rgb[2]);
            wsum += wi;
        }
    }
    const double PI = 3.14159265358979323846;
    const float phi = (float)(0.5 * PI - ((double)r + 0.5) * (PI / (double)h));
    const float theta = (float)(PI - ((double)c + 0.5) * (2.0 * PI / (double)w));
    const float cp = cosf(phi);
    float4* o = reinterpret_cast<float4*>(cells + 8 * (size_t)t);
    o[0] = make_float4(cosf(theta) * cp, sinf(theta) * cp, sinf(phi), (float)b * rows);
    o[1] = make_float4(rgb[0] / wsum, rgb[1] / wsum, rgb[2] / wsum, 0.f);
}

struct LightShadow {
    const float* pts;
    const float* frames;
    const uint32_t* maps;
    int S;
    tir::ShadowBias bias;
};

template <bool SHADOW>
__device__ __forceinline__ void light_rows(const float4* __restrict__ gbuf, const float* __restrict__ view, const float4* __restrict__ cells,
                                           int64_t M, int D, float fresnel, int flags, float4* __restrict__ out, const LightShadow& sh) {
    const int64_t m = (int64_t)blockIdx.x * blockDim.x + threadIdx.x;
    if (m >= M) return;
    const float4 g0 = gbuf[3 * m], g1 = gbuf[3 * m + 1], g2 = gbuf[3 * m + 2];
    const float cov = g2.x;
    if (!(cov > 0.f)) { out[m] = make_float4(0.f, 0.f, 0.f, 0.f); return; }
    const float rough = g0.w, ao = g1.x;
    const float ns[3] = {g1.y, g1.z, g1.w};
    const float rough3[3] = {rough, rough, rough}, fres3[3] = {fresnel, fresnel, fresnel}, alb[3] = {g0.x, g0.y, g0.z};
    const Surface s = make_surface(ns, view + 3 * m, rough3, fres3, alb);
    const float alpha2 = s.alpha2[0], k = s.k[0], omk = 1.f - k, omf = 1.f - fresnel;
    const float nom1 = s.NoV * omk + k;
    const float four_pi = 4.0f * 3.14159265358979323846f;
    float acc[3] = {0.f, 0.f, 0.f};
    float pt[3] = {0.f, 0.f, 0.f};
    if constexpr (SHADOW) { pt[0] = sh.pts[3 * m]; pt[1] = sh.pts[3 * m + 1]; pt[2] = sh.pts[3 * m + 2]; }
    for (int d = 0; d < D; ++d) {
        const float4 ca = cells[2 * (size_t)d], cb = cells[2 * (size_t)d + 1];
        const float lx = ca.x, ly = ca.y, lz = ca.z;
        const float c = ns[0] * lx + ns[1] * ly + ns[2] * lz;
        if (c > 1e-6f) {
            if constexpr (SHADOW) {
                if (!tir::shadow_lit(sh.frames + 12 * (size_t)d, sh.maps + (size_t)d * (size_t)sh.S * (size_t)sh.S, sh.S, pt[0], pt[1],
                                     pt[2], c, sh.bias))
                    continue;
            }
            float hx = (lx + s.V[0]) * 0.5f, hy = (ly + s.V[1]) * 0.5f, hz = (lz + s.V[2]) * 0.5f;
            const float inv = __builtin_amdgcn_rsqf(fmaxf(hx * hx + hy * hy + hz * hz, 1e-24f));
            hx *= inv; hy *= inv; hz *= inv;
            const float NoL = fminf(fmaxf(s.N[0] * lx + s.N[1] * ly + s.N[2] * lz, 1e-6f), 1.f);
            const float NoH = fminf(fmaxf(s.N[0] * hx + s.N[1] * hy + s.N[2] * hz, 1e-6f), 1.f);
            const float VoH = fminf(fmaxf(s.V[0] * hx + s.V[1] * hy + s.V[2] * hz, 1e-6f), 1.f);
            const float p2 = __builtin_amdgcn_exp2f(((-5.55473f) * VoH - 6.98316f) * VoH);
            const float frac = (fresnel + omf * p2) * alpha2;
            const float nom0 = NoH * NoH * (alpha2 - 1.f) + 1.f;
            const float nom2 = NoL * omk + k;
            const float nom = fminf(fmaxf(four_pi * nom0 * nom0 * nom1 * nom2, 1e-6f), four_pi);
            const float spec = frac * __builtin_amdgcn_rcpf(nom);
            acc[0] += (s.alb_pi[0] + spec) * cb.x * c * ca.w;
            acc[1] += (s.alb_pi[1] + spec) * cb.y * c * ca.w;
            acc[2] += (s.alb_pi[2] + spec) * cb.z * c * ca.w;
        }
    }
#pragma unroll
    for (int q = 0; q < 3; ++q) {
        if (flags & TIR_LIGHT_OCCLUSION) acc[q] *= ao;
        if (flags & TIR_LIGHT_SRGB) acc[q] = linear2srgb(acc[q]);
    }
    out[m] = make_float4(acc[0], acc[1], acc[2], cov);
}

__global__ void __launch_bounds__(256)
k_light_gbuffer(const float4* __restrict__ gbuf, const float* __restrict__ view, const float4* __restrict__ cells, int64_t M, int D,
                float fresnel, int flags, float4* __restrict__ out) {
    light_rows<false>(gbuf, view, cells, M, D, fresnel, flags, out, LightShadow{});
}

__global__ void __launch_bounds__(256)
k_light_gbuffer_shadowed(const float4* __restrict__ gbuf, const float* __restrict__ view, const float4* __restrict__ cells, int64_t M,
                         int D, float fresnel, int flags, float4* __restrict__ out, LightShadow sh) {
    light_rows<true>(gbuf, view, cells, M, D, fresnel, flags, out, sh);
}

}

extern "C" int tir_env_cells(const float* hdr, int32_t H, int32_t W, const float* row_w, int32_t h, int32_t w, float* cells,
                             void* stream) {
    if (H < 1 || W < 1 || h < 1 || w < 1 || H % h != 0 || W % w != 0) return TIR_ERR_ARG;
    if (!hdr || !row_w || !cells || reinterpret_cast<uintptr_t>(cells) % 16 != 0) return TIR_ERR_ARG;
    if ((int64_t)H * W > ((int64_t)1 << 28)) return TIR_ERR_UNSUPPORTED;
    const int64_t n = (int64_t)h * w;
    hipLaunchKernelGGL(k_env_cells, dim3((unsigned)((n + 255) / 256)), dim3(256), 0, tir_stream(stream), hdr, H, W, row_w, h, w,
                       cells);
    TIR_CHECK_LAUNCH();
    return TIR_OK;
}

extern "C" int tir_light_gbuffer(const float* gbuf, const float* view, const float* cells, int64_t M, int32_t D, float fresnel,
                                 int32_t flags, float* out, void* stream) {
    if (M < 0 || D < 1 || (flags & ~(TIR_LIGHT_OCCLUSION | TIR_LIGHT_SRGB))) return TIR_ERR_ARG;
    if (D > (1 << 20) || M > ((int64_t)1 << 36)) return TIR_ERR_UNSUPPORTED;
    if (M == 0) return TIR_OK;
    if (!gbuf || !view || !cells || !out) return TIR_ERR_ARG;
    if (reinterpret_cast<uintptr_t>(gbuf) % 16 != 0 || reinterpret_cast<uintptr_t>(cells) % 16 != 0 ||
        reinterpret_cast<uintptr_t>(out) % 16 != 0)
        return TIR_ERR_ARG;
    hipLaunchKernelGGL(k_light_gbuffer, dim3((unsigned)((M + 255) / 256)), dim3(256), 0, tir_stream(stream),
                       reinterpret_cast<const float4*>(gbuf), view, reinterpret_cast<const float4*>(cells), M, (int)D, fresnel,
                       (int)flags, reinterpret_cast<float4*>(out));
    TIR_CHECK_LAUNCH();
    return TIR_OK;
}

extern "C" int tir_light_gbuffer_shadowed(const float* gbuf, const float* view, const float* cells, const float* pts, const float* frames,
                                          const uint32_t* maps, int64_t M, int32_t D, int32_t S, float bias_const, float bias_slope,
                                          float fresnel, int32_t flags, float* out, void* stream) {
    if (M < 0 || D < 1 || S < 1 || (flags & ~(TIR_LIGHT_OCCLUSION | TIR_LIGHT_SRGB))) return TIR_ERR_ARG;
    if (!(bias_const >= 0.f && bias_const < INFINITY) || !(bias_slope >= 0.f && bias_slope < INFINITY)) return TIR_ERR_ARG;
    if (D > (1 << 20) || M > ((int64_t)1 << 36) || S > TIR_SHADOW_MAX_SIDE) return TIR_ERR_UNSUPPORTED;
    if (M == 0) return TIR_OK;
    if (!gbuf || !view || !cells || !out || !pts || !frames || !maps) return TIR_ERR_ARG;
    if (reinterpret_cast<uintptr_t>(gbuf) % 16 != 0 || reinterpret_cast<uintptr_t>(cells) % 16 != 0 ||
        reinterpret_cast<uintptr_t>(out) % 16 != 0 || reinterpret_cast<uintptr_t>(frames) % 16 != 0 ||
        reinterpret_cast<uintptr_t>(maps) % 4 != 0)
        return TIR_ERR_ARG;
    const LightShadow sh{pts, frames, maps, (int)S, tir::ShadowBias{bias_const, bias_slope, 0.5f / (float)S}};
    hipLaunchKernelGGL(k_light_gbuffer_shadowed, dim3((unsigned)((M + 255) / 256)), dim3(256), 0, tir_stream(stream),
                       reinterpret_cast<const float4*>(gbuf), view, reinterpret_cast<const float4*>(cells), M, (int)D, fresnel,
                       (int)flags, reinterpret_cast<float4*>(out), sh);
    TIR_CHECK_LAUNCH();
    return TIR_OK;
}

extern "C" int tir_env_sg_fwd(const TirEnvSG* e, const float* dirs, int32_t D, float* out, void* stream) {
    if (!e || !e->sgs || !e->rot || e->n_sg <= 0 || e->n_lights <= 0 || D < 0) return TIR_ERR_ARG;
    if (D == 0) return TIR_OK;
    if (!dirs || !out) return TIR_ERR_ARG;
    hipLaunchKernelGGL(k_env_sg, dim3(e->n_lights * D), dim3(128), 0, tir_stream(stream), *e, dirs, D, out);
    TIR_CHECK_LAUNCH();
    return TIR_OK;
}

extern "C" int tir_shade_setup(const float* maps, const float* rays, const float* dirs, int32_t M,
                               int32_t D, float acc_thres, float* surf, uint8_t* active, void* stream) {
    if (M < 0 || D <= 0) return TIR_ERR_ARG;
    if (M == 0) return TIR_OK;
    if (!maps || !rays || !dirs || !surf || !active) return TIR_ERR_ARG;
    int64_t n = (int64_t)M * D;
    hipLaunchKernelGGL(k_shade_setup, dim3((unsigned)((n + 255) / 256)), dim3(256), 0, tir_stream(stream), maps,
                       rays, dirs, M, D, acc_thres, surf, active, (int32_t*)nullptr, (int32_t*)nullptr, (float*)nullptr,
                       (int32_t*)nullptr, 0);
    TIR_CHECK_LAUNCH();
    return TIR_OK;
}

extern "C" int tir_shade_setup_compact(const float* maps, const float* rays, const float* dirs, int32_t M,
                                       int32_t D, float acc_thres, float* surf, uint8_t* active, int32_t* pair_ids,
                                       int32_t* n_active, float* vis, int32_t* ray_rec_cnt, int32_t pair_order, void* stream) {
    if (M < 0 || D <= 0) return TIR_ERR_ARG;
    if (M == 0) return TIR_OK;
    if (!maps || !rays || !dirs || !surf || !active || !pair_ids || !n_active) return TIR_ERR_ARG;
    int64_t n = (int64_t)M * D;
    if (n >= ((int64_t)1 << 31)) return TIR_ERR_UNSUPPORTED;
    if (pair_order < 0 || pair_order > 2) return TIR_ERR_ARG;
    const int dir_major = pair_order == 2 ? 0 : 1;
    hipLaunchKernelGGL(k_shade_setup, dim3((unsigned)((n + 1023) / 1024)), dim3(1024), 0, tir_stream(stream), maps,
                       rays, dirs, M, D, acc_thres, surf, active, pair_ids, n_active, vis, ray_rec_cnt, dir_major);
    TIR_CHECK_LAUNCH();
    return TIR_OK;
}

extern "C" int tir_shade_integrate(const float* maps, const float* rays, const float* dirs,
                                   const int32_t* light_idx, const float* vis, const float* indirect,
                                   const float* env, const float* weight_d, int32_t M, int32_t D,
                                   int32_t n_lights, int32_t equal_area, int32_t use_srgb, float acc_thres,
                                   float* out_rgb, void* stream) {
    if (M < 0 || D <= 0 || n_lights <= 0) return TIR_ERR_ARG;
    if (M == 0) return TIR_OK;
    if (!maps || !rays || !dirs || !vis || !env || !out_rgb || (!equal_area && !weight_d)) return TIR_ERR_ARG;
    hipLaunchKernelGGL(k_shade_integrate, dim3((M + 3) / 4), dim3(256), 0, tir_stream(stream), maps, rays, dirs,
                       light_idx, vis, indirect, env, weight_d, M, D, n_lights, equal_area, use_srgb, acc_thres, out_rgb,
                       (const int32_t*)nullptr, (const int32_t*)nullptr, (const float*)nullptr, (const float*)nullptr,
                       (int32_t*)nullptr);
    TIR_CHECK_LAUNCH();
    return TIR_OK;
}

extern "C" int tir_shade_integrate_records(const float* maps, const float* rays, const float* dirs,
                                           const int32_t* light_idx, const float* vis, const int32_t* ray_rec_off,
                                           const int32_t* ray_rec_cnt, const float* rec_w, const float* rec_rgb,
                                           const float* env, const float* weight_d, int32_t M, int32_t D,
                                           int32_t n_lights, int32_t equal_area, int32_t use_srgb, float acc_thres,
                                           float* out_rgb, int32_t* reset_counter, void* stream) {
    if (M < 0 || D <= 0 || n_lights <= 0) return TIR_ERR_ARG;
    if (M == 0) return TIR_OK;
    if (!maps || !rays || !dirs || !vis || !env || !out_rgb || (!equal_area && !weight_d)) return TIR_ERR_ARG;
    if (!ray_rec_off || !ray_rec_cnt || !rec_w || !rec_rgb) return TIR_ERR_ARG;
    hipLaunchKernelGGL(k_shade_integrate, dim3((M + 3) / 4), dim3(256), 0, tir_stream(stream), maps, rays, dirs,
                       light_idx, vis, (const float*)nullptr, env, weight_d, M, D, n_lights, equal_area, use_srgb,
                       acc_thres, out_rgb, ray_rec_off, ray_rec_cnt, rec_w, rec_rgb, reset_counter);
    TIR_CHECK_LAUNCH();
    return TIR_OK;
}

extern "C" int tir_relight_importance(const float* normal, const float* albedo, const float* rough,
                                      const float* fresnel, const float* rays_d, const float* light_dir,
                                      const float* light_rgb, const float* light_pdf, const float* vis,
                                      int32_t M, int32_t Ns, float* out_rgb, void* stream) {
    if (M < 0 || Ns <= 0) return TIR_ERR_ARG;
    if (M == 0) return TIR_OK;
    if (!normal || !albedo || !rough || !fresnel || !rays_d || !light_dir || !light_rgb || !light_pdf || !vis || !out_rgb)
        return TIR_ERR_ARG;
    hipLaunchKernelGGL(k_relight_importance, dim3((M + 3) / 4), dim3(256), 0, tir_stream(stream), normal, albedo,
                       rough, fresnel, rays_d, light_dir, light_rgb, light_pdf, vis, M, Ns, out_rgb);
    TIR_CHECK_LAUNCH();
    return TIR_OK;
}

extern "C" int tir_env_sample_setup(const float* row_cdf, const float* col_cdf, int32_t H, int32_t W, const float* env_dir,
                                    const float* normal, int32_t M, int32_t Ns, uint64_t seed, uint64_t offset,
                                    int32_t* cell, uint8_t* active, void* stream) {
    if (M < 0 || Ns <= 0 || H <= 0 || W <= 0) return TIR_ERR_ARG;
    if (M == 0) return TIR_OK;
    if (!row_cdf || !col_cdf || !env_dir || !normal || !cell || !active) return TIR_ERR_ARG;
    const int64_t n = (int64_t)M * Ns;
    hipLaunchKernelGGL(k_env_sample_setup, dim3((unsigned)((n + 255) / 256)), dim3(256), 0, tir_stream(stream), row_cdf,
                       col_cdf, H, W, env_dir, normal, M, Ns, (unsigned long long)seed, (unsigned long long)offset, cell, active);
    TIR_CHECK_LAUNCH();
    return TIR_OK;
}

extern "C" int tir_env_sample_setup_list_n(const float* row_cdf, const float* col_cdf, int32_t H, int32_t W, const float* env_dir,
                                           int32_t dir_stride, const float* normal, int32_t M, int32_t Ns, uint64_t seed, uint64_t offset,
                                           int32_t bins_r, int32_t bins_c, int32_t block_pairs, const int32_t* row_guide,
                                           const uint16_t* col_guide, int32_t guide_rows, int32_t guide_cols, int32_t* cell,
                                           float* vis, int32_t* pair_ids, int32_t* n_active, const int32_t* m_dev, void* stream) {
    if (M < 0 || Ns <= 0 || H <= 0 || W <= 0 || bins_r <= 0 || bins_c <= 0 || dir_stride < 3) return TIR_ERR_ARG;
    if ((row_guide == nullptr) != (col_guide == nullptr)) return TIR_ERR_ARG;
    if (row_guide) {
        if (guide_rows <= 0 || guide_cols <= 0 || (guide_rows & (guide_rows - 1)) || (guide_cols & (guide_cols - 1))) return TIR_ERR_ARG;
        if (W > 65535 || guide_rows > (1 << 20) || guide_cols > (1 << 20)) return TIR_ERR_UNSUPPORTED;
    }
    if ((int64_t)bins_r * bins_c > 255 || block_pairs < 256 || block_pairs > 32768) return TIR_ERR_UNSUPPORTED;
    if (M == 0) return TIR_OK;
    if (!row_cdf || !col_cdf || !env_dir || !normal || !cell || !vis || !pair_ids || !n_active) return TIR_ERR_ARG;
    const int64_t n = (int64_t)M * Ns;
    if (n >= (int64_t)1 << 31) return TIR_ERR_UNSUPPORTED;
    const size_t lds = (size_t)block_pairs * 3;
    if (int rc = tir_allow_dynamic_lds(reinterpret_cast<const void*>(k_env_sample_list), 100 * 1024)) return rc;
    hipLaunchKernelGGL(k_env_sample_list, dim3((unsigned)((n + block_pairs - 1) / block_pairs)), dim3(256), lds,
                       tir_stream(stream), row_cdf, col_cdf, H, W, env_dir, dir_stride, normal, M, Ns, (unsigned long long)seed,
                       (unsigned long long)offset, bins_r, bins_c, block_pairs, row_guide, col_guide, guide_rows, guide_cols, cell,
                       vis, pair_ids, n_active, m_dev);
    TIR_CHECK_LAUNCH();
    return TIR_OK;
}

extern "C" int tir_env_sample_setup_list(const float* row_cdf, const float* col_cdf, int32_t H, int32_t W, const float* env_dir,
                                         int32_t dir_stride, const float* normal, int32_t M, int32_t Ns, uint64_t seed, uint64_t offset,
                                         int32_t bins_r, int32_t bins_c, int32_t block_pairs, const int32_t* row_guide,
                                         const uint16_t* col_guide, int32_t guide_rows, int32_t guide_cols, int32_t* cell,
                                         float* vis, int32_t* pair_ids, int32_t* n_active, void* stream) {
    return tir_env_sample_setup_list_n(row_cdf, col_cdf, H, W, env_dir, dir_stride, normal, M, Ns, seed, offset, bins_r, bins_c, block_pairs,
                                       row_guide, col_guide, guide_rows, guide_cols, cell, vis, pair_ids, n_active, nullptr, stream);
}

extern "C" int tir_relight_importance_cells(const float* normal, const float* albedo, const float* rough,
                                            const float* fresnel, const float* rays_d, const int32_t* cell,
                                            const float* env_dir, const float* env_rgb, const float* env_pdf,
                                            const float* vis, int32_t M, int32_t Ns, float* out_rgb, void* stream) {
    if (M < 0 || Ns <= 0) return TIR_ERR_ARG;
    if (M == 0) return TIR_OK;
    if (!normal || !albedo || !rough || !fresnel || !rays_d || !cell || !env_dir || !env_rgb || !env_pdf || !vis || !out_rgb)
        return TIR_ERR_ARG;
    hipLaunchKernelGGL(k_relight_importance_cells<false>, dim3((M + 3) / 4), dim3(256), 0, tir_stream(stream), normal, albedo,
                       rough, fresnel, rays_d, cell, env_dir, env_rgb, env_pdf, vis, M, Ns, out_rgb, nullptr);
    TIR_CHECK_LAUNCH();
    return TIR_OK;
}

extern "C" int tir_relight_importance_cells_packed_n(const float* normal, const float* albedo, const float* rough,
                                                     const float* fresnel, const float* rays_d, const int32_t* cell,
                                                     const float* env_cell, const float* vis, int32_t M, int32_t Ns,
                                                     float* out_rgb, const int32_t* m_dev, void* stream) {
    if (M < 0 || Ns <= 0) return TIR_ERR_ARG;
    if (M == 0) return TIR_OK;
    if (!normal || !albedo || !rough || !fresnel || !rays_d || !cell || !env_cell || !vis || !out_rgb) return TIR_ERR_ARG;
    if (reinterpret_cast<uintptr_t>(env_cell) % 16 != 0) return TIR_ERR_ARG;
    hipLaunchKernelGGL(k_relight_importance_cells<true>, dim3((M + 3) / 4), dim3(256), 0, tir_stream(stream), normal, albedo,
                       rough, fresnel, rays_d, cell, env_cell, nullptr, nullptr, vis, M, Ns, out_rgb, m_dev);
    TIR_CHECK_LAUNCH();
    return TIR_OK;
}

extern "C" int tir_relight_importance_cells_packed(const float* normal, const float* albedo, const float* rough,
                                                   const float* fresnel, const float* rays_d, const int32_t* cell,
                                                   const float* env_cell, const float* vis, int32_t M, int32_t Ns,
                                                   float* out_rgb, void* stream) {
    return tir_relight_importance_cells_packed_n(normal, albedo, rough, fresnel, rays_d, cell, env_cell, vis, M, Ns, out_rgb, nullptr, stream);
}

extern "C" int tir_env_lookup(const float* env_rgb, int32_t H, int32_t W, const float* dirs, int64_t n, float* out,
                              void* stream) {
    if (n < 0 || H <= 0 || W <= 0) return TIR_ERR_ARG;
    if (n == 0) return TIR_OK;
    if (!env_rgb || !dirs || !out) return TIR_ERR_ARG;
    hipLaunchKernelGGL(k_env_lookup, dim3((unsigned)((n + 255) / 256)), dim3(256), 0, tir_stream(stream), env_rgb, H, W,
                       dirs, 3, n, out, 3, nullptr, nullptr);
    TIR_CHECK_LAUNCH();
    return TIR_OK;
}

extern "C" int tir_env_compose(const float* env_rgb, int32_t H, int32_t W, const float* dirs, int32_t dir_stride, int64_t n,
                               const int32_t* slot, const float* fg_rgb, float* out, int32_t out_stride, void* stream) {
    if (n < 0 || H <= 0 || W <= 0 || dir_stride < 3 || out_stride < 3) return TIR_ERR_ARG;
    if (n == 0) return TIR_OK;
    if (!env_rgb || !dirs || !out || !slot || !fg_rgb) return TIR_ERR_ARG;
    hipLaunchKernelGGL(k_env_lookup, dim3((unsigned)((n + 255) / 256)), dim3(256), 0, tir_stream(stream), env_rgb, H, W,
                       dirs, dir_stride, n, out, out_stride, slot, fg_rgb);
    TIR_CHECK_LAUNCH();
// ... 76 lines not shown
```

tensoir_amd/field_model.py:

```python
from __future__ import annotations

import functools
import math
import time

import numpy as np
import torch
import torch.nn as nn
import torch.nn.functional as F

from . import capacity, indirect, ops, regularisers
from ._lib import TensoirHipError, TirField

MAT_MODE = [[0, 1], [0, 2], [1, 2]]
VEC_MODE = [2, 1, 0]


def raw2alpha(sigma, dist):
    alpha = 1.0 - torch.exp(-sigma * dist)
    T = torch.cumprod(torch.cat([torch.ones(alpha.shape[0], 1).to(alpha.device), 1.0 - alpha + 1e-10], -1), -1)
    weights = alpha * T[:, :-1]
    return alpha, weights, T[:, -1:]


# ... 754 lines not shown
        keep = [slice(int(a), int(b)) for a, b in zip(first, last)]
        cropped = lambda t: nn.Parameter(channel_last(t))
        for i, ((m0, m1), v) in enumerate(zip(self.matMode, self.vecMode)):
            for lines, planes in ((self.density_line, self.density_plane), (self.app_line, self.app_plane)):
                lines[i] = cropped(lines[i].data[..., keep[v], :])
                planes[i] = cropped(planes[i].data[..., keep[m1], keep[m0]])
        if not torch.all(self.alphaMask.gridSize == self.gridSize):
            lo_frac, hi_frac = first / (self.gridSize - 1), (last - 1) / (self.gridSize - 1)
            lo, hi = self.aabb[0], self.aabb[1]
            new_aabb = torch.stack([(1 - lo_frac) * lo + lo_frac * hi, (1 - hi_frac) * lo + hi_frac * hi]).to(new_aabb.dtype)
        self.aabb = new_aabb
        self.update_stepSize(tuple(last - first))

    def get_kwargs(self):
        return {"aabb": self.aabb, "gridSize": self.gridSize.tolist(), **{k: getattr(self, a) for k, a in _CKPT_KWARGS.items()}}

    def save(self, path):
        ckpt = {"kwargs": self.get_kwargs(), "state_dict": self.state_dict()}
        if self.alphaMask is not None:
            occupied = self.alphaMask.alpha_volume.bool().cpu().numpy()
            ckpt["alphaMask.shape"] = occupied.shape
            ckpt["alphaMask.mask"] = np.packbits(occupied.reshape(-1))
            ckpt["alphaMask.aabb"] = self.alphaMask.aabb.cpu()
        torch.save(ckpt, path)
        try:
            import json
            with open(str(path) + ".tensoir_amd.json", "w") as fh:
                json.dump({"indirect_precision": self.indirect_precision()}, fh, indent=1, default=str)
        except OSError:
            pass

    def load(self, ckpt):
        if "alphaMask.aabb" in ckpt:
            shape = tuple(ckpt["alphaMask.shape"])
            bits = np.unpackbits(ckpt["alphaMask.mask"])[:int(np.prod(shape))]
            self.alphaMask = AlphaGridMask(self.device, ckpt["alphaMask.aabb"].to(self.device),
                                           torch.from_numpy(bits.reshape(shape)).float().to(self.device))
        self.load_state_dict(ckpt["state_dict"])
        self._field_key = None
        indirect.reset(self)

    def forward(self, rays_chunk, light_idx, white_bg=True, is_train=False, ndc_ray=False, is_relight=True,
                N_samples=-1, _brdf_jitter_dense=None, _return_maps=False, _defer_check=False, _want_mask=True):
        if ndc_ray:
            raise NotImplementedError("ndc_ray=True is not on the TensoIR hot path (no shipped config uses it)")
        dev = rays_chunk.device
        rays = rays_chunk.to(torch.float32).contiguous()
        B = rays.shape[0]
        S = N_samples if N_samples > 0 else self.nSamples
        f = self.packed_field()
        lidx = ops.to_device(light_idx.reshape(-1), dev, torch.int32).contiguous()
        jitter = ops.to_device(torch.rand(B, 1), dev) if is_train else None
        from . import training
        if training.wants_grad(self):
            bg = bool(white_bg or (is_train and torch.rand((1,)) < 0.5))
            for attempt in range(2):
                try:
                    maps = training.PrimaryRenderFn.apply(self, rays, lidx, S, bg, bool(is_relight), jitter,
                                                          _brdf_jitter_dense, bool(_defer_check),
                                                          *training.field_param_list(self))
                    break
                except training._CapacityOverflow:
                    if attempt:
                        raise
            out = self.unpack_maps(maps, is_relight, want_mask=_want_mask)
            return (out, maps) if _return_maps else out
        rc = capacity.PassCapacity(self.__dict__.setdefault("_app_cap_hints", {}), (B, S), 1.25, ceiling=B * S, max_entries=64,
                                   capture=self.__dict__.get("_capture"), check_key=("primary", B, S))
        cap = rc.hinted() if (not is_train and _brdf_jitter_dense is None) else None
        words = viewdirs = None
        if cap is None:
            weight, acc, depth, _tend, cnt = ops.march_primary(f, rays, jitter, S, self.march_t_stop)
            offsets = ops.exclusive_scan(cnt)
            A, n_dev = int(offsets[-1].item()), None
        else:
            words = self._step_words(dev)
            weight, acc, depth, cnt, offsets, total_dev, viewdirs = ops.march_primary_fused(f, rays, S, self.march_t_stop,
                                                                                            cap, words)
            self.__dict__["_rec_counter_armed"] = words[1:3]
            A, n_dev = cap, offsets[B:]
            rc.watch(total_dev, cap)
        rec_ray, rec_k, rec_w, rec_xyz = ops.compact_primary(f, rays, jitter, weight, offsets, A)
        rgb = brdf = brdf_j = pred = derived = None
        rng_state = None
        if A > 0:
            if viewdirs is None:
                viewdirs = rays[:, 3:6].contiguous()
            merged = bool(is_relight) and _brdf_jitter_dense is None and f.n_acomp == 48 and ops.APP_IMPL == "mfma"
            if merged:
                rng_state = self._jitter_rng(dev)
                rad, intr, xyz_j, intr_j = ops.vm_app_primary(f, rec_xyz, lidx, rec_ray, 0.01, rng_state, n_dev)
            else:
                rad, intr = ops.vm_app(f, rec_xyz, lidx, rec_ray, True, bool(is_relight), None, 0, n_dev)
            jobs = [(self.renderModule.packed(), rad, viewdirs, rec_ray)]
            if is_relight:
                pb = self.renderModule_brdf.packed()
                jobs.append((pb, intr, rec_xyz, None))
                if merged:
                    pass
                elif _brdf_jitter_dense is not None:
                    noise = _brdf_jitter_dense.to(dev, torch.float32)[rec_ray.long(), rec_k.long()]
                    xyz_j = torch.add(rec_xyz, noise, alpha=0.01)
                    intr_j = ops.vm_app(f, xyz_j, None, None, False, True, None, 0, n_dev)[1]
                else:
                    rng_state = self._jitter_rng(dev)
                    xyz_j, intr_j = ops.vm_app_jitter(f, rec_xyz, 0.01, 0, 0, rng_state, n_dev)
                jobs.append((pb, intr_j, xyz_j, None))
                if self.normals_kind in ("purely_predicted", "derived_plus_predicted"):
                    jobs.append((self.renderModule_normal.packed(), intr, rec_xyz, None))
            if ops.MLP_IMPL == "bf16x3":
                outs = ops.mlp_multi(jobs, n_dev)
            else:
                outs = [ops.mlp(m, ft, ax, mp, None, 0, n_dev) for m, ft, ax, mp in jobs]
            rgb = outs[0]
            if is_relight:
                brdf, brdf_j = outs[1], outs[2]
                if self.normals_kind == "purely_derived":
                    pred = ops.density_grad(f, rec_xyz, n_dev=n_dev)[2]
                elif self.normals_kind == "gt_normals":
                    pred = None
                elif self.normals_kind == "residue_prediction":
                    derived = ops.density_grad(f, rec_xyz, n_dev=n_dev)[2]
                    pred = self.renderModule_normal.rows(rec_xyz, derived, intr, n_dev)
                else:
                    pred = outs[3]
                    if self.normals_kind == "derived_plus_predicted":
                        derived = ops.density_grad(f, rec_xyz, n_dev=n_dev)[2]
        bg = bool(white_bg or (is_train and torch.rand((1,)) < 0.5))
        smooth = None
        if words is not None:
            maps, smooth = ops.composite_primary_fused(rays, offsets, rec_w, rgb, brdf, brdf_j, pred, derived, acc, depth,
                                                       bg, is_relight, self.fixed_fresnel, words, rng_state, 1)
        else:
            maps = ops.composite_primary(rays, offsets, rec_w, rgb, brdf, brdf_j, pred, derived, acc, depth,
                                         bg, is_relight, self.fixed_fresnel)
            if rng_state is not None:
                rng_state[1] += 1
        if self.normals_kind not in NORMAL_LOSS_KINDS and is_relight:
            maps[:, 16] = 0.0

        if rc.capture is None:
            finish = rc.settle if words is not None else functools.partial(rc.settle, A)
            if _defer_check:
                self.__dict__["_pending_primary"] = finish
            elif not finish():
                return self.forward(rays_chunk, light_idx, white_bg, is_train, ndc_ray, is_relight, N_samples,
                                    _brdf_jitter_dense, _return_maps, False, _want_mask)
        out = self.unpack_maps(maps, is_relight, want_mask=_want_mask, smooth=smooth)
        return (out, maps) if _return_maps else out

    def _step_words(self, dev):
        w = self.__dict__.get("_words")
        if w is None or w.device != torch.device(dev):
            w = self.__dict__["_words"] = torch.zeros((8,), dtype=torch.int32, device=dev)
            self.__dict__["_pair_counter"] = w[0:1]
        return w

    def _jitter_rng(self, dev):
        seed = int(torch.cuda.initial_seed())
        st = self.__dict__.get("_jit_rng")
        if st is None or st[0] != seed or st[1].device != torch.device(dev):
            if self.__dict__.get("_capture") is not None:
                raise TensoirHipError("the jitter RNG state must exist before a graph capture (run one eager call first)")
            t = torch.tensor([seed & (2 ** 63 - 1), 0], dtype=torch.int64).to(dev)
            st = self.__dict__["_jit_rng"] = (seed, t)
        return st[1]

    def _finish_primary(self):
        fin = self.__dict__.pop("_pending_primary", None)
        return True if fin is None else fin()

    @staticmethod
    def unpack_maps(maps, is_relight=True, want_mask=True, smooth=None):
        if not is_relight:
            return (maps[:, 0:3], maps[:, 3], None, None, None, None, maps[:, 14], None, None, None, None, None)
        if maps.requires_grad:
            rgb, depth, normal, albedo, rough, fresnel, acc, ndiff, norient, sm, _pad = torch.split(
                maps, [3, 1, 3, 3, 1, 3, 1, 1, 1, 2, 1], dim=1)
            depth, acc = depth.squeeze(-1), acc.squeeze(-1)
            if smooth is None:
                smooth = torch.mean(sm, dim=0)
            return (rgb, depth, normal, albedo, rough, fresnel, acc, ndiff, norient, (acc > 0.5) if want_mask else None,
                    smooth[0], smooth[1])
        acc = maps[:, 14]
        if smooth is None:
            smooth = torch.mean(maps[:, 17:19], dim=0)
        return (maps[:, 0:3], maps[:, 3], maps[:, 4:7], maps[:, 7:10], maps[:, 10:11], maps[:, 11:14], acc,
                maps[:, 15:16], maps[:, 16:17], (acc > 0.5) if want_mask else None, smooth[0], smooth[1])
```

tensoir_amd/ops.py:

```python
from __future__ import annotations

import ctypes as C
import math
import os

import numpy as np
import torch

from . import _lib
from ._lib import TirEnvSG, TirField, TirFieldHalf, TirMlp, check, lib

MAP_STRIDE = 20

STATS = None
TIMING = None

TUNE = {
    "lds_lines": 2 if os.environ.get("TENSOIR_LDS_LINES", "1") == "0" else 0,
    "xcd_order": 1 if os.environ.get("TIR_XCD", "0") == "1" else 0,
    "dense_sigma": 0 if os.environ.get("TENSOIR_DENSE_SIGMA", "1") == "0" else 1,
    "dense_sigma_max_mb": max(0, int(os.environ.get("TENSOIR_DENSE_SIGMA_MAX_MB", "1024") or 0)),
    "mlp_grid": max(0, int(os.environ.get("TENSOIR_MLP_GRID", "0") or 0)),
    "pair_order": 2 if os.environ.get("TIR_PAIR_ORDER", "d")[:1] == "m" else 0,
    "wgrad_blocks": max(0, int(os.environ.get("TENSOIR_WGRAD_BLOCKS", "0") or 0)),
# ... 385 lines not shown

def indirect_fused(field: TirField, fh: TirFieldHalf, m: "PackedMlp", xyz, light_idx, rec_map, idx_div, dirs, n_dirs, n_dev=None):
    xyz = f32(xyz, "xyz", 3).view(-1, 3)
    n = xyz.shape[0]
    light_idx = i32(light_idx, "light_idx").view(-1)
    rec_map = i32(rec_map, "rec_map").view(-1)
    if rec_map.numel() != n:
        raise ValueError("rec_map must have one entry per record")
    dirs = f32(dirs, "dirs", 3)
    table = _aux_table_cached(m, dirs)
    out = torch.empty((n, m.out_dim), dtype=torch.float32, device=xyz.device)
    _call("tir_indirect_fused_fwd", C.byref(field), C.byref(fh), C.byref(m.desc), _ptr(xyz), _ptr(light_idx), _ptr(rec_map), int(idx_div),
          int(n_dirs), _ptr(table), _ptr(out), n, _ptr(n_dev), _stream())
    return out


def indirect_fused_hp(field: TirField, m: "PackedMlp", xyz, light_idx, rec_map, idx_div, dirs, n_dirs, n_dev=None):
    xyz = f32(xyz, "xyz", 3).view(-1, 3)
    n = xyz.shape[0]
    light_idx = i32(light_idx, "light_idx").view(-1)
    rec_map = i32(rec_map, "rec_map").view(-1)
    if rec_map.numel() != n:
        raise ValueError("rec_map must have one entry per record")
    dirs = f32(dirs, "dirs", 3)
    table = _aux_table_cached(m, dirs)
    out = torch.empty((n, m.out_dim), dtype=torch.float32, device=xyz.device)
    _call("tir_indirect_fused_hp_fwd", C.byref(field), C.byref(m.desc), _ptr(xyz), _ptr(light_idx), _ptr(rec_map), int(idx_div),
          int(n_dirs), _ptr(table), _ptr(out), n, _ptr(n_dev), _stream())
    return out


MLP_ENTRY = {"mfma": "tir_mlp_fwd", "bf16x3": "tir_mlp_fwd_bf16x3", "bf16": "tir_mlp_fwd_bf16",
             "valu": "tir_mlp_fwd_valu"}
MLP_IMPL = os.environ.get("TENSOIR_DECODER", "bf16x3")
if MLP_IMPL not in MLP_ENTRY:
    raise ValueError(f"TENSOIR_DECODER={MLP_IMPL!r}: expected one of {sorted(MLP_ENTRY)}")
_IND = os.environ.get("TENSOIR_INDIRECT_PRECISION", "auto")
if _IND not in ("auto", "f16", "hp", "full"):
    raise ValueError(f"TENSOIR_INDIRECT_PRECISION={_IND!r}: expected auto, f16, hp or full")
SECONDARY_MLP_IMPL = {"full": None, "hp": "hp"}.get(_IND, "f16")
SECONDARY_APP_IMPL = "h16" if _IND in ("auto", "f16") else None
INDIRECT_GUARD = _IND == "auto"
INDIRECT_HP = os.environ.get("TENSOIR_INDIRECT_HP", "1") != "0"
INDIRECT_PROBE = {"map_limit": float(os.environ.get("TENSOIR_INDIRECT_MAP_LIMIT", "2.5e-5")), "train_map_limit": 1.0e-4, "records": 32768, "interval": 64, "w_bias": 0.5, "w_rms": 0.25, "w_max": 0.25, "limit": 2.5e-5,
                  "range": 6.0e4}


FUSED_INDIRECT = os.environ.get("TENSOIR_FUSED_INDIRECT", "1") != "0"


def fused_indirect():
    return FUSED_INDIRECT and AUX_TABLE and secondary_app_impl() == "h16" and secondary_mlp_impl() == "f16"


def full_indirect_route():
    gather = "tir_vm_app_fwd_x3 (fp32 taps, fp16 hi + lo contraction)" if app_contraction() == "x3" else "tir_vm_app_fwd (fp32 taps, fp32 MFMA contraction)"
    return gather + " + tir_mlp_fwd_auxtab_bf16x3 (split-bf16 x3), feature rows through HBM"


def hp_indirect_route():
    return ("tir_indirect_fused_hp_fwd: fp32 taps, fp16 hi + lo basis contraction, decoder with fp16 activations and fp16 + fp8-residue "
            "weights (residue on the block-scaled fp8 matrix instruction), one launch, feature rows in registers")


def secondary_app_impl():
    return SECONDARY_APP_IMPL if (MLP_IMPL == "bf16x3" and SECONDARY_APP_IMPL) else None


def secondary_mlp_impl():
    return SECONDARY_MLP_IMPL if (MLP_IMPL == "bf16x3" and SECONDARY_MLP_IMPL) else None


def mlp_multi(jobs, n_dev=None, save_hidden=False):
    n = jobs[0][1].shape[0]
    k = len(jobs)
    feats, auxs, maps, outs = [], [], [], []
    for m, feat, aux, aux_map in jobs:
        feat = f32(feat, "feat")
        if feat.shape[0] != n or feat.dim() != 2 or feat.shape[1] != FEAT_STRIDE:
            raise ValueError(f"mlp_multi: every job needs [n, {FEAT_STRIDE}] feature rows")
        aux = f32(aux, "aux", 3)
        if aux_map is not None:
            aux_map = i32(aux_map, "aux_map").view(-1)
        elif aux.shape[0] != n:
            raise ValueError("aux must have one row per feature row (or pass aux_map)")
        feats.append(feat); auxs.append(aux); maps.append(aux_map)
        outs.append(torch.empty((n, m.out_dim), dtype=torch.float32, device=feat.device))
    arr = lambda ts: (C.c_void_p * k)(*[None if t is None else t.data_ptr() for t in ts])
    descs = (C.POINTER(TirMlp) * k)(*[C.pointer(m.desc) for m, _, _, _ in jobs])
    use_tab = [AUX_TABLE and AUX_TABLE_MULTI and not save_hidden and mp is not None and aux.shape[0] * 8 <= max(n, 1)
               for aux, mp in zip(auxs, maps)]
    if any(use_tab):
        tables = [mlp_aux_table(m, aux) if t else None for (m, _, _, _), aux, t in zip(jobs, auxs, use_tab)]
        _call("tir_mlp_fwd_multi_auxtab_bf16x3", descs, arr(feats), FEAT_STRIDE, arr(auxs), arr(maps), arr(tables), arr(outs), k, n,
              _ptr(n_dev), _stream())
        return outs
    if save_hidden:
        h1s = [torch.empty((n, 128), dtype=torch.float32, device=outs[0].device) for _ in range(k)]
        h2s = [torch.empty((n, 128), dtype=torch.float32, device=outs[0].device) for _ in range(k)]
        _call("tir_mlp_train_fwd_multi_bf16x3", descs, arr(feats), FEAT_STRIDE, arr(auxs), arr(maps), arr(outs), arr(h1s), arr(h2s),
              k, n, _ptr(n_dev), _stream())
        return list(zip(outs, h1s, h2s))
    _call("tir_mlp_fwd_multi_bf16x3", descs, arr(feats), FEAT_STRIDE, arr(auxs), arr(maps), arr(outs), k, n, _ptr(n_dev),
          _stream())
    return outs


def mlp(m: PackedMlp, feat, aux, aux_map=None, impl=None, aux_mod=0, n_dev=None):
    impl = impl or MLP_IMPL
    feat = f32(feat, "feat")
    if feat.dim() != 2 or feat.shape[1] < m.desc.feat_dim:
        raise ValueError(f"feat: expected [n, >= {m.desc.feat_dim}], got {tuple(feat.shape)}")
    aux = f32(aux, "aux", 3)
    n = feat.shape[0]
    if aux_map is not None:
        aux_map = i32(aux_map, "aux_map").view(-1)
        if aux_map.numel() != n:
            raise ValueError("aux_map must have one entry per row")
    elif aux.shape[0] != n and aux_mod <= 0:
        raise ValueError("aux must have one row per feature row")
    out = torch.empty((n, m.out_dim), dtype=torch.float32, device=feat.device)
    f16 = impl == "f16"
    if f16:
        impl = "bf16x3"
    if impl == "bf16x3" and AUX_TABLE and (aux_map is not None or aux_mod > 0) and aux.shape[0] * 8 <= max(n, 1):
        table = _aux_table_cached(m, aux)
        _call("tir_mlp_fwd_auxtab_f16" if f16 else "tir_mlp_fwd_auxtab_bf16x3", C.byref(m.desc), _ptr(feat), feat.shape[1], _ptr(table),
              _ptr(aux_map), int(aux_mod), _ptr(out), n, _ptr(n_dev), _stream())
        return out
    _call(MLP_ENTRY[impl], C.byref(m.desc), _ptr(feat), feat.shape[1], _ptr(aux),
          _ptr(aux_map), int(aux_mod), _ptr(out), n, _ptr(n_dev), _stream())
    return out


def march_primary(field: TirField, rays, ray_jitter, n_samples, t_stop):
    rays = f32(rays, "rays", 6)
    B = rays.shape[0]
    dev = rays.device
    if ray_jitter is not None:
        ray_jitter = f32(ray_jitter, "ray_jitter").view(-1)
        if ray_jitter.numel() != B:
            raise ValueError("ray_jitter must be [B] / [B,1]")
    weight = torch.empty((B, n_samples), dtype=torch.float32, device=dev)
    acc = torch.empty((B,), dtype=torch.float32, device=dev)
    depth = torch.empty((B,), dtype=torch.float32, device=dev)
    tend = torch.empty((B,), dtype=torch.float32, device=dev)
    cnt = torch.empty((B,), dtype=torch.int32, device=dev)
    _call("tir_march_primary_fwd", C.byref(field), _ptr(rays), _ptr(ray_jitter), B, n_samples,
                                      float(t_stop), _ptr(weight), _ptr(acc), _ptr(depth), _ptr(tend),
                                      _ptr(cnt), _stats_ptr("tir_march_primary_fwd", dev), _stream())
    return weight, acc, depth, tend, cnt


def march_primary_fused(field: TirField, rays, n_samples, t_stop, cap, words):
    rays = f32(rays, "rays", 6)
    B = rays.shape[0]
    dev = rays.device
    weight = torch.empty((B, n_samples), dtype=torch.float32, device=dev)
    acc = torch.empty((B,), dtype=torch.float32, device=dev)
    depth = torch.empty((B,), dtype=torch.float32, device=dev)
    cnt = torch.empty((B,), dtype=torch.int32, device=dev)
    off = torch.empty((B + 1,), dtype=torch.int32, device=dev)
    vd = torch.empty((B, 3), dtype=torch.float32, device=dev)
    total = words[5:6]
    _call("tir_march_primary_fused_fwd", C.byref(field), _ptr(rays), None, B, n_samples, float(t_stop), _ptr(weight),
          _ptr(acc), _ptr(depth), None, _ptr(cnt), _stats_ptr("tir_march_primary_fwd", dev), _ptr(vd),
          C.c_void_p(words.data_ptr() + 4), 2, C.c_void_p(words.data_ptr() + 12), _ptr(off), int(cap), _ptr(total), _stream())
    return weight, acc, depth, cnt, off, total, vd


def composite_primary_fused(rays, offsets, rec_w, rgb, brdf, brdf_jit, pred_n, der_n, acc, depth, white_bg, is_relight,
                            fixed_fresnel, words, rng_state=None, rng_step=0):
    rays = f32(rays, "rays", 6)
    B = rays.shape[0]
    out = torch.empty((B, MAP_STRIDE), dtype=torch.float32, device=rays.device)
    smooth = torch.zeros((2,), dtype=torch.float32, device=rays.device) if B == 0 else \
        torch.empty((2,), dtype=torch.float32, device=rays.device)
    _call("tir_composite_primary_fused", _ptr(rays), _ptr(offsets), _ptr(rec_w), _ptr(rgb), _ptr(brdf), _ptr(brdf_jit),
          _ptr(pred_n), _ptr(der_n), _ptr(acc), _ptr(depth), B, int(bool(white_bg)), int(bool(is_relight)),
          float(fixed_fresnel), _ptr(out), C.c_void_p(words.data_ptr() + 16), _ptr(smooth), _ptr(rng_state), int(rng_step),
          _stream())
    return out, smooth


def vm_app_jitter(field: TirField, xyz, scale, seed, offset, rng_state=None, n_dev=None):
    xyz = f32(xyz, "xyz", 3).view(-1, 3)
    n = xyz.shape[0]
    xyz_j = torch.empty_like(xyz)
    intr = torch.empty((n, FEAT_STRIDE), dtype=torch.float32, device=xyz.device)
    _call("tir_vm_app_jitter_fwd", C.byref(field), _ptr(xyz), n, _ptr(n_dev), float(scale), int(seed) & (2 ** 64 - 1),
          int(offset) & (2 ** 64 - 1), _ptr(rng_state), _ptr(xyz_j), _ptr(intr), FEAT_STRIDE, _stream())
    return xyz_j, intr


APP_CONTRACTION = os.environ.get("TENSOIR_APP_CONTRACTION", "fp32")
if APP_CONTRACTION not in ("x3", "fp32"):
    raise ValueError(f"TENSOIR_APP_CONTRACTION={APP_CONTRACTION!r}: expected x3 or fp32")


def app_contraction():
    return APP_CONTRACTION if MLP_IMPL == "bf16x3" else "fp32"


def vm_app_primary(field: TirField, xyz, light_idx, idx_map, scale, rng_state, n_dev=None, exact=False):
    xyz = f32(xyz, "xyz", 3).view(-1, 3)
    n = xyz.shape[0]
    dev = xyz.device
    rad = torch.empty((n, FEAT_STRIDE), dtype=torch.float32, device=dev)
    intr = torch.empty((n, FEAT_STRIDE), dtype=torch.float32, device=dev)
    intr_j = torch.empty((n, FEAT_STRIDE), dtype=torch.float32, device=dev)
    xyz_j = torch.empty_like(xyz)
    _call("tir_vm_app_primary_fwd" if (exact or app_contraction() == "fp32") else "tir_vm_app_primary_x3_fwd", C.byref(field), _ptr(xyz),
          _ptr(i32(light_idx, "light_idx").view(-1)),
          _ptr(None if idx_map is None else i32(idx_map, "idx_map").view(-1)), _ptr(rad), _ptr(intr), FEAT_STRIDE, n, _ptr(n_dev),
          float(scale), 0, 0, _ptr(rng_state), _ptr(xyz_j), _ptr(intr_j), _stream())
    return rad, intr, xyz_j, intr_j


def exclusive_scan(counts):
    counts = i32(counts, "counts").view(-1)
    n = counts.numel()
    off = torch.empty((n + 1,), dtype=torch.int32, device=counts.device)
    _call("tir_exclusive_scan", _ptr(counts), _ptr(off), n, _stream())
    return off


def exclusive_scan_capped(counts, cap):
    counts = i32(counts, "counts").view(-1)
    n = counts.numel()
    off = torch.empty((n + 1,), dtype=torch.int32, device=counts.device)
    total = torch.empty((1,), dtype=torch.int32, device=counts.device)
    _call("tir_exclusive_scan_capped", _ptr(counts), _ptr(off), n, int(cap), _ptr(total), _stream())
    return off, total


def compact_primary(field: TirField, rays, ray_jitter, weight, offsets, total):
    rays = f32(rays, "rays", 6)
    B, S = weight.shape
    dev = rays.device
    if ray_jitter is not None:
        ray_jitter = f32(ray_jitter, "ray_jitter").view(-1)
    rec_ray = torch.empty((total,), dtype=torch.int32, device=dev)
    rec_k = torch.empty((total,), dtype=torch.int32, device=dev)
    rec_w = torch.empty((total,), dtype=torch.float32, device=dev)
    rec_xyz = torch.empty((total, 3), dtype=torch.float32, device=dev)
    if total > 0:
        _call("tir_compact_primary", C.byref(field), _ptr(rays), _ptr(ray_jitter), _ptr(weight),
                                        _ptr(offsets), B, S, _ptr(rec_ray), _ptr(rec_k), _ptr(rec_w),
                                        _ptr(rec_xyz), _stream())
    return rec_ray, rec_k, rec_w, rec_xyz


def composite_primary(rays, offsets, rec_w, rgb, brdf, brdf_jit, pred_n, der_n, acc, depth,
                      white_bg, is_relight, fixed_fresnel):
    rays = f32(rays, "rays", 6)
    B = rays.shape[0]
    out = torch.empty((B, MAP_STRIDE), dtype=torch.float32, device=rays.device)
    _call("tir_composite_primary", _ptr(rays), _ptr(offsets), _ptr(rec_w), _ptr(rgb), _ptr(brdf),
                                      _ptr(brdf_jit), _ptr(pred_n), _ptr(der_n), _ptr(acc), _ptr(depth),
                                      B, int(bool(white_bg)), int(bool(is_relight)),
                                      float(fixed_fresnel), _ptr(out), _stream())
    return out


def march_secondary(field: TirField, origins, dirs, z_vals, n_rays, org_map=None, dir_map=None,
                    active=None, t_stop=0.0, want_records=False, rec_cap=0, want_nerfactor=True, n_dirs=0,
                    ray_ids=None, n_ids_dev=None, vis=None, rec_cnt=None, counter=None):
    origins = f32(origins, "origins", 3)
    dirs = f32(dirs, "dirs", 3)
    z_vals = f32(z_vals, "z_vals").view(-1)
    dev = origins.device
    n_sample = z_vals.numel()
    org_map = None if org_map is None else i32(org_map, "org_map")
    dir_map = None if dir_map is None else i32(dir_map, "dir_map")
    if active is not None:
        active = _req(active, torch.uint8, "active")
    if vis is None:
        vis = torch.empty((n_rays,), dtype=torch.float32, device=dev)
    oma = torch.empty((n_rays,), dtype=torch.float32, device=dev) if want_nerfactor else None
    rec = None
    if want_records:
        rec = {
            "counter": counter if counter is not None else torch.zeros((2,), dtype=torch.int32, device=dev),
            "ray": torch.empty((rec_cap,), dtype=torch.int32, device=dev),
            "w": torch.empty((rec_cap,), dtype=torch.float32, device=dev),
            "xyz": torch.empty((rec_cap, 3), dtype=torch.float32, device=dev),
            "off": torch.empty((n_rays,), dtype=torch.int32, device=dev),
            "cnt": rec_cnt if rec_cnt is not None else torch.empty((n_rays,), dtype=torch.int32, device=dev),
            "cap": rec_cap,
        }
    r = rec or {}
    if ray_ids is not None:
        ray_ids = i32(ray_ids, "ray_ids")
    _call("tir_march_secondary_fwd" if ray_ids is None else "tir_march_secondary_ids_fwd",
          C.byref(field), _ptr(origins), _ptr(org_map), _ptr(dirs), _ptr(dir_map), _ptr(active),
          n_rays, int(n_dirs), n_sample, _ptr(z_vals), float(t_stop), _ptr(vis), _ptr(oma),
          _ptr(r.get("counter")), int(rec_cap), _ptr(r.get("ray")), _ptr(r.get("w")), _ptr(r.get("xyz")),
          _ptr(r.get("off")), _ptr(r.get("cnt")), _stats_ptr("tir_march_secondary_fwd", dev),
          *(() if ray_ids is None else (_ptr(ray_ids), _ptr(n_ids_dev))), _stream())
    return vis, oma, rec


def accumulate_records(off, cnt, rec_w, rec_rgb, n_rays):
    out = torch.empty((n_rays, 3), dtype=torch.float32, device=off.device)
    _call("tir_accumulate_records", _ptr(off), _ptr(cnt), _ptr(rec_w), _ptr(rec_rgb), n_rays,
                                       _ptr(out), _stream())
    return out


def env_sg(lgtSGs, rot, dirs):
    sgs = f32(lgtSGs.detach(), "lgtSGs", 7)
    rot = f32(rot, "light_rotation_matrix").view(-1, 9)
    dirs = f32(dirs, "dirs", 3).view(-1, 3)
    L, D = rot.shape[0], dirs.shape[0]
    out = torch.empty((L, D, 3), dtype=torch.float32, device=dirs.device)
    desc = TirEnvSG(sgs.data_ptr(), rot.data_ptr(), sgs.shape[0], L)
    _call("tir_env_sg_fwd", C.byref(desc), _ptr(dirs), D, _ptr(out), _stream())
    return out


def env_pixel(light_rgbs, H, W, rot, dirs, softplus=True):
    lr = f32(light_rgbs.detach(), "_light_rgbs", 3).view(-1, 3)
    if lr.shape[0] != H * W:
        raise ValueError(f"_light_rgbs: expected {H * W} rows, got {lr.shape[0]}")
    rot = f32(rot, "light_rotation_matrix").view(-1, 9)
    dirs = f32(dirs, "dirs", 3).view(-1, 3)
    L, D = rot.shape[0], dirs.shape[0]
    out = torch.empty((L, D, 3), dtype=torch.float32, device=dirs.device)
    _call("tir_env_pixel_fwd", _ptr(lr), int(H), int(W), _ptr(rot), _ptr(dirs), L, D, int(bool(softplus)), _ptr(out), _stream())
    return out


def env_pixel_bwd(light_rgbs, H, W, rot, dirs, g_env):
# ... 1089 lines not shown
```

Baseline: 4.981 million.

## Use two-level grouped completion tickets and multi-pair shade setup blocks

Replaces the single global last-block ticket counter in the fused primary march and composite kernels with a two-level scheme: blocks first increment one of 32 cache-line-separated group counters, and only the last block of each group touches the root counter. This is meant to reduce atomic contention on a single word across thousands of workgroups. Separately, the shade setup compaction kernel now processes two pairs per thread and replaces the serial per-block prefix over wave counts with a wave-wide shuffle scan, halving block count and global atomics. The step-words buffer grows to hold the ticket lines, and the dir-major path recomputes activity per pair, which adds extra loads.

```diff
diff --git a/include/tensoir_hip.h b/include/tensoir_hip.h
--- a/include/tensoir_hip.h
+++ b/include/tensoir_hip.h
@@ -194,6 +194,14 @@
                                 float* viewdirs, int32_t* zero_words, int32_t n_zero, int32_t* ticket,
                                 int32_t* offsets, int32_t cap, int32_t* total, void* stream);
 
+#define TIR_STEP_TICKET_WORDS 1056
+
+int tir_march_primary_fused2_fwd(const TirField* f, const float* rays, const float* ray_jitter,
+                                 int32_t B, int32_t S, float t_stop, float* weight, float* acc,
+                                 float* depth, float* t_end, int32_t* app_count, unsigned long long* stats,
+                                 float* viewdirs, int32_t* zero_words, int32_t n_zero, int32_t* tickets,
+                                 int32_t* offsets, int32_t cap, int32_t* total, void* stream);
+
 int tir_exclusive_scan(const int32_t* counts, int32_t* offsets, int32_t n, void* stream);
 int tir_exclusive_scan_capped(const int32_t* counts, int32_t* offsets, int32_t n, int32_t cap,
                               int32_t* total, void* stream);
@@ -220,6 +228,12 @@
                                 int32_t is_relight, float fixed_fresnel, float* out_maps, int32_t* ticket,
                                 float* smooth_out, int64_t* rng_state, int64_t rng_step, void* stream);
 
+int tir_composite_primary_fused2(const float* rays, const int32_t* offsets, const float* rec_w,
+                                 const float* rgb, const float* brdf, const float* brdf_jit,
+                                 const float* pred_normal, const float* derived_normal,
+                                 const float* acc, const float* depth, int32_t B, int32_t white_bg,
+                                 int32_t is_relight, float fixed_fresnel, float* out_maps, int32_t* tickets,
+                                 float* smooth_out, int64_t* rng_state, int64_t rng_step, void* stream);
 
 int tir_march_secondary_fwd(const TirField* f, const float* origins, const int32_t* org_map,
                             const float* dirs, const int32_t* dir_map, const uint8_t* active,
@@ -255,6 +269,7 @@
 int tir_shade_setup_compact(const float* maps, const float* rays, const float* dirs, int32_t M,
                             int32_t D, float acc_thres, float* surf, uint8_t* active, int32_t* pair_ids,
                             int32_t* n_active, float* vis, int32_t* ray_rec_cnt, int32_t pair_order, void* stream);
+int tir_shade_setup_segment(void);
 
 int tir_shade_integrate(const float* maps, const float* rays, const float* dirs,
                         const int32_t* light_idx, const float* vis, const float* indirect,
diff --git a/tensoir_amd/_lib.py b/tensoir_amd/_lib.py
--- a/tensoir_amd/_lib.py
+++ b/tensoir_amd/_lib.py
@@ -97,6 +97,9 @@
     "tir_march_primary_fused_fwd": (C.c_int, [C.POINTER(TirField), P, P, I32, I32, F32, P, P, P, P, P, P,
                                               P, P, I32, P, P, I32, P, P]),
     "tir_composite_primary_fused": (C.c_int, [P, P, P, P, P, P, P, P, P, P, I32, I32, I32, F32, P, P, P, P, I64, P]),
+    "tir_march_primary_fused2_fwd": (C.c_int, [C.POINTER(TirField), P, P, I32, I32, F32, P, P, P, P, P, P,
+                                               P, P, I32, P, P, I32, P, P]),
+    "tir_composite_primary_fused2": (C.c_int, [P, P, P, P, P, P, P, P, P, P, I32, I32, I32, F32, P, P, P, P, I64, P]),
     "tir_vm_app_jitter_fwd": (C.c_int, [C.POINTER(TirField), P, I64, P, F32, C.c_uint64, C.c_uint64, P, P, P, I32, P]),
     "tir_vm_app_primary_fwd": (C.c_int, [C.POINTER(TirField), P, P, P, P, P, I32, I64, P, F32, C.c_uint64, C.c_uint64, P, P, P, P]),
     "tir_vm_app_primary_x3_fwd": (C.c_int, [C.POINTER(TirField), P, P, P, P, P, I32, I64, P, F32, C.c_uint64, C.c_uint64, P, P, P, P]),
@@ -112,6 +115,7 @@
     "tir_shade_integrate": (C.c_int, [P, P, P, P, P, P, P, P, I32, I32, I32, I32, I32, F32, P, P]),
     "tir_shade_integrate_records": (C.c_int, [P, P, P, P, P, P, P, P, P, P, P, I32, I32, I32, I32, I32, F32, P, P, P]),
     "tir_shade_setup_compact": (C.c_int, [P, P, P, I32, I32, F32, P, P, P, P, P, P, I32, P]),
+    "tir_shade_setup_segment": (C.c_int, []),
     "tir_march_secondary_ids_fwd": (C.c_int, [C.POINTER(TirField), P, P, P, P, P, I64, I32, I32, P, F32, P, P,
                                               P, I64, P, P, P, P, P, P, P, P, P]),
     "tir_relight_importance": (C.c_int, [P, P, P, P, P, P, P, P, P, I32, I32, P, P]),
diff --git a/tensoir_amd/csrc/tir_common.hpp b/tensoir_amd/csrc/tir_common.hpp
--- a/tensoir_amd/csrc/tir_common.hpp
+++ b/tensoir_amd/csrc/tir_common.hpp
@@ -853,4 +853,27 @@
     return *s_last != 0;
 }
 
-}
+#define TIR_TICKET_GROUPS 32
+#define TIR_TICKET_LINE 32
+#define TIR_TICKET_WORDS ((TIR_TICKET_GROUPS + 1) * TIR_TICKET_LINE)
+#if TIR_TICKET_WORDS != TIR_STEP_TICKET_WORDS
+#error "TIR_STEP_TICKET_WORDS of tensoir_hip.h must equal the ticket layout of tir_common.hpp"
+#endif
+
+__device__ __forceinline__ bool draw_ticket(int32_t* word, int expected) {
+    const int t = __hip_atomic_fetch_add(word, 1, __ATOMIC_RELAXED, __HIP_MEMORY_SCOPE_AGENT);
+    if (t != expected - 1) return false;
+    __hip_atomic_store(word, 0, __ATOMIC_RELAXED, __HIP_MEMORY_SCOPE_AGENT);
+    return true;
+}
+
+__device__ __forceinline__ bool last_workgroup_ticket(int32_t* ticket, bool two_level) {
+    const int blocks = (int)gridDim.x;
+    if (!two_level) return draw_ticket(ticket, blocks);
+    const int g = (int)blockIdx.x % TIR_TICKET_GROUPS;
+    const int members = (blocks - g + TIR_TICKET_GROUPS - 1) / TIR_TICKET_GROUPS;
+    if (!draw_ticket(ticket + (1 + g) * TIR_TICKET_LINE, members)) return false;
+    return draw_ticket(ticket, min(blocks, TIR_TICKET_GROUPS));
+}
+
+}
diff --git a/tensoir_amd/csrc/tir_march.hip b/tensoir_amd/csrc/tir_march.hip
--- a/tensoir_amd/csrc/tir_march.hip
+++ b/tensoir_amd/csrc/tir_march.hip
@@ -73,6 +73,7 @@
     float* viewdirs;
     int32_t* zero_words; int n_zero;
     int32_t* ticket; int32_t* offsets; int cap; int32_t* total_out;
+    int ticket_two_level;
 };
 
 __device__ __forceinline__ void block_exclusive_scan_capped(const int32_t* __restrict__ counts, int32_t* __restrict__ offsets,
@@ -135,11 +136,7 @@
     __shared__ int s_last;
     asm volatile("s_waitcnt vmcnt(0)" ::: "memory");
     __syncthreads();
-    if (threadIdx.x == 0) {
-        const int t = __hip_atomic_fetch_add(ex.ticket, 1, __ATOMIC_RELAXED, __HIP_MEMORY_SCOPE_AGENT);
-        s_last = (t == (int)gridDim.x - 1);
-        if (s_last) __hip_atomic_store(ex.ticket, 0, __ATOMIC_RELAXED, __HIP_MEMORY_SCOPE_AGENT);
-    }
+    if (threadIdx.x == 0) s_last = last_workgroup_ticket(ex.ticket, ex.ticket_two_level != 0);
     __syncthreads();
     if (s_last) block_exclusive_scan_capped(app_count, ex.offsets, B, ex.cap, ex.total_out);
 }
@@ -159,22 +156,40 @@
     return TIR_OK;
 }
 
-extern "C" int tir_march_primary_fused_fwd(const TirField* f, const float* rays, const float* ray_jitter,
-                                           int32_t B, int32_t S, float t_stop, float* weight, float* acc,
-                                           float* depth, float* t_end, int32_t* app_count, unsigned long long* stats,
-                                           float* viewdirs, int32_t* zero_words, int32_t n_zero, int32_t* ticket,
-                                           int32_t* offsets, int32_t cap, int32_t* total, void* stream) {
+static int march_primary_fused(const TirField* f, const float* rays, const float* ray_jitter,
+                               int32_t B, int32_t S, float t_stop, float* weight, float* acc,
+                               float* depth, float* t_end, int32_t* app_count, unsigned long long* stats,
+                               float* viewdirs, int32_t* zero_words, int32_t n_zero, int32_t* ticket, int two_level,
+                               int32_t* offsets, int32_t cap, int32_t* total, void* stream) {
     if (!f || B < 0 || S <= 0 || n_zero < 0 || n_zero > 256 || cap < 0) return TIR_ERR_ARG;
     if ((ticket == nullptr) != (offsets == nullptr)) return TIR_ERR_ARG;
     if (B == 0) return TIR_OK;
     if (!rays || !weight || !acc || !depth || !app_count) return TIR_ERR_ARG;
     if (!(f->n_dcomp == 4 || f->n_dcomp == 8 || f->n_dcomp == 16 || f->n_dcomp == 32)) return TIR_ERR_UNSUPPORTED;
     if (!tir_occ_index_ok(f) || !tir_plane_index_ok(f)) return TIR_ERR_UNSUPPORTED;
-    TirMarchExtras ex{viewdirs, zero_words, n_zero, ticket, offsets, cap, total};
+    TirMarchExtras ex{viewdirs, zero_words, n_zero, ticket, offsets, cap, total, two_level};
     hipLaunchKernelGGL(k_march_primary, dim3((B + 3) / 4), dim3(256), 0, tir_stream(stream), *f, rays,
                        ray_jitter, B, S, t_stop, weight, acc, depth, t_end, app_count, stats, (float*)nullptr, ex);
     TIR_CHECK_LAUNCH();
     return TIR_OK;
+}
+
+extern "C" int tir_march_primary_fused_fwd(const TirField* f, const float* rays, const float* ray_jitter,
+                                           int32_t B, int32_t S, float t_stop, float* weight, float* acc,
+                                           float* depth, float* t_end, int32_t* app_count, unsigned long long* stats,
+                                           float* viewdirs, int32_t* zero_words, int32_t n_zero, int32_t* ticket,
+                                           int32_t* offsets, int32_t cap, int32_t* total, void* stream) {
+    return march_primary_fused(f, rays, ray_jitter, B, S, t_stop, weight, acc, depth, t_end, app_count, stats, viewdirs,
+                               zero_words, n_zero, ticket, 0, offsets, cap, total, stream);
+}
+
+extern "C" int tir_march_primary_fused2_fwd(const TirField* f, const float* rays, const float* ray_jitter,
+                                            int32_t B, int32_t S, float t_stop, float* weight, float* acc,
+                                            float* depth, float* t_end, int32_t* app_count, unsigned long long* stats,
+                                            float* viewdirs, int32_t* zero_words, int32_t n_zero, int32_t* tickets,
+                                            int32_t* offsets, int32_t cap, int32_t* total, void* stream) {
+    return march_primary_fused(f, rays, ray_jitter, B, S, t_stop, weight, acc, depth, t_end, app_count, stats, viewdirs,
+                               zero_words, n_zero, tickets, 1, offsets, cap, total, stream);
 }
 
 extern "C" int tir_march_primary_train_fwd(const TirField* f, const float* rays, const float* ray_jitter,
@@ -323,6 +338,7 @@
 
 struct TirCompositeExtras {
     int32_t* ticket; float* smooth_out;
+    int ticket_two_level;
     long long* rng_bump; long long rng_step;
 };
 
@@ -438,11 +454,7 @@
     __shared__ float s_part[2][4];
     asm volatile("s_waitcnt vmcnt(0)" ::: "memory");
     __syncthreads();
-    if (threadIdx.x == 0) {
-        const int t = __hip_atomic_fetch_add(ex.ticket, 1, __ATOMIC_RELAXED, __HIP_MEMORY_SCOPE_AGENT);
-        s_last = (t == (int)gridDim.x - 1);
-        if (s_last) __hip_atomic_store(ex.ticket, 0, __ATOMIC_RELAXED, __HIP_MEMORY_SCOPE_AGENT);
-    }
+    if (threadIdx.x == 0) s_last = last_workgroup_ticket(ex.ticket, ex.ticket_two_level != 0);
     __syncthreads();
     if (!s_last) return;
     float a = 0.0f, g = 0.0f;
@@ -474,21 +486,41 @@
     return TIR_OK;
 }
 
+static int composite_primary_fused(const float* rays, const int32_t* offsets, const float* rec_w,
+                                   const float* rgb, const float* brdf, const float* brdf_jit,
+                                   const float* pred_normal, const float* derived_normal,
+                                   const float* acc, const float* depth, int32_t B, int32_t white_bg,
+                                   int32_t is_relight, float fixed_fresnel, float* out_maps, int32_t* ticket, int two_level,
+                                   float* smooth_out, int64_t* rng_state, int64_t rng_step, void* stream) {
+    if (B < 0 || (ticket == nullptr) != (smooth_out == nullptr)) return TIR_ERR_ARG;
+    if (B == 0) return TIR_OK;
+    if (!rays || !offsets || !acc || !depth || !out_maps) return TIR_ERR_ARG;
+    TirCompositeExtras ex{ticket, smooth_out, two_level, reinterpret_cast<long long*>(rng_state), (long long)rng_step};
+    hipLaunchKernelGGL(k_composite_primary, dim3((B + 3) / 4), dim3(256), 0, tir_stream(stream), rays, offsets,
+                       rec_w, rgb, brdf, brdf_jit, pred_normal, derived_normal, acc, depth, B, white_bg,
+                       is_relight, fixed_fresnel, out_maps, ex);
+    TIR_CHECK_LAUNCH();
+    return TIR_OK;
+}
+
 extern "C" int tir_composite_primary_fused(const float* rays, const int32_t* offsets, const float* rec_w,
                                            const float* rgb, const float* brdf, const float* brdf_jit,
                                            const float* pred_normal, const float* derived_normal,
                                            const float* acc, const float* depth, int32_t B, int32_t white_bg,
                                            int32_t is_relight, float fixed_fresnel, float* out_maps, int32_t* ticket,
                                            float* smooth_out, int64_t* rng_state, int64_t rng_step, void* stream) {
-    if (B < 0 || (ticket == nullptr) != (smooth_out == nullptr)) return TIR_ERR_ARG;
-    if (B == 0) return TIR_OK;
-    if (!rays || !offsets || !acc || !depth || !out_maps) return TIR_ERR_ARG;
-    TirCompositeExtras ex{ticket, smooth_out, reinterpret_cast<long long*>(rng_state), (long long)rng_step};
-    hipLaunchKernelGGL(k_composite_primary, dim3((B + 3) / 4), dim3(256), 0, tir_stream(stream), rays, offsets,
-                       rec_w, rgb, brdf, brdf_jit, pred_normal, derived_normal, acc, depth, B, white_bg,
-                       is_relight, fixed_fresnel, out_maps, ex);
-    TIR_CHECK_LAUNCH();
-    return TIR_OK;
+    return composite_primary_fused(rays, offsets, rec_w, rgb, brdf, brdf_jit, pred_normal, derived_normal, acc, depth, B,
+                                   white_bg, is_relight, fixed_fresnel, out_maps, ticket, 0, smooth_out, rng_state, rng_step, stream);
+}
+
+extern "C" int tir_composite_primary_fused2(const float* rays, const int32_t* offsets, const float* rec_w,
+                                            const float* rgb, const float* brdf, const float* brdf_jit,
+                                            const float* pred_normal, const float* derived_normal,
+                                            const float* acc, const float* depth, int32_t B, int32_t white_bg,
+                                            int32_t is_relight, float fixed_fresnel, float* out_maps, int32_t* tickets,
+                                            float* smooth_out, int64_t* rng_state, int64_t rng_step, void* stream) {
+    return composite_primary_fused(rays, offsets, rec_w, rgb, brdf, brdf_jit, pred_normal, derived_normal, acc, depth, B,
+                                   white_bg, is_relight, fixed_fresnel, out_maps, tickets, 1, smooth_out, rng_state, rng_step, stream);
 }
 
 #define TIR_SEC_MAX_SAMPLES 256
diff --git a/tensoir_amd/csrc/tir_shade.hip b/tensoir_amd/csrc/tir_shade.hip
--- a/tensoir_amd/csrc/tir_shade.hip
+++ b/tensoir_amd/csrc/tir_shade.hip
@@ -91,49 +91,104 @@
     }
 }
 
+#ifndef TIR_SETUP_PAIRS
+#define TIR_SETUP_PAIRS 2
+#endif
+
+__device__ __forceinline__ bool pair_active(const float* __restrict__ maps, const float* __restrict__ dirs, int m, int d,
+                                            float acc_thres) {
+    const float* mp = maps + (size_t)m * TIR_MAP_STRIDE;
+    float cs = dirs[3 * d] * mp[4] + dirs[3 * d + 1] * mp[5] + dirs[3 * d + 2] * mp[6];
+    return fmaxf(cs, 0.f) > 1e-6f && mp[14] > acc_thres;
+}
+
+template <int P>
 __global__ void __launch_bounds__(1024)
 k_shade_setup(const float* __restrict__ maps, const float* __restrict__ rays, const float* __restrict__ dirs,
               int M, int D, float acc_thres, float* __restrict__ surf, uint8_t* __restrict__ active,
               int32_t* __restrict__ pair_ids, int32_t* __restrict__ n_active, float* __restrict__ vis,
               int32_t* __restrict__ rec_cnt, int dir_major) {
-    const int64_t t = (int64_t)blockIdx.x * blockDim.x + threadIdx.x;
-    const bool in = t < (int64_t)M * D;
-    int64_t i = t;
-    if (dir_major && in) i = (t % M) * D + t / M;
-    bool act = false;
-    if (in) {
-        const int m = (int)(i / D), d = (int)(i % D);
-        const float* mp = maps + (size_t)m * TIR_MAP_STRIDE;
-        const float* r = rays + 6 * (size_t)m;
-        if (d == 0) {
-            const float depth = mp[3];
-#pragma unroll
-            for (int a = 0; a < 3; ++a) surf[3 * (size_t)m + a] = add_rn(r[a], mul_rn(depth, r[3 + a]));
-        }
-        float cs = dirs[3 * d] * mp[4] + dirs[3 * d + 1] * mp[5] + dirs[3 * d + 2] * mp[6];
-        act = fmaxf(cs, 0.f) > 1e-6f && mp[14] > acc_thres;
-        active[i] = act ? 1 : 0;
+    const int64_t n = (int64_t)M * D;
+    const int64_t t0 = (int64_t)blockIdx.x * ((int64_t)blockDim.x * P) + threadIdx.x;
+    int64_t idx[P];
+    bool act[P];
+#pragma unroll
+    for (int j = 0; j < P; ++j) {
+        const int64_t t = t0 + (int64_t)j * blockDim.x;
+        idx[j] = t;
+        act[j] = false;
+        if (t < n) {
+            const int m = (int)(t / D), d = (int)(t % D);
+            if (d == 0) {
+                const float* mp = maps + (size_t)m * TIR_MAP_STRIDE;
+                const float* r = rays + 6 * (size_t)m;
+                const float depth = mp[3];
+#pragma unroll
+                for (int a = 0; a < 3; ++a) surf[3 * (size_t)m + a] = add_rn(r[a], mul_rn(depth, r[3 + a]));
+            }
+            act[j] = pair_active(maps, dirs, m, d, acc_thres);
+            active[t] = act[j] ? 1 : 0;
+            if (pair_ids && !act[j]) {
+                if (vis) vis[t] = 0.0f;
+                if (rec_cnt) rec_cnt[t] = 0;
+            }
+        }
     }
     if (!pair_ids) return;
-    __shared__ int s_wcnt[16];
+    if (dir_major) {
+#pragma unroll
+        for (int j = 0; j < P; ++j) {
+            const int64_t t = t0 + (int64_t)j * blockDim.x;
+            if (t < n) {
+                const int m = (int)(t % M), d = (int)(t / M);
+                idx[j] = (int64_t)m * D + d;
+                act[j] = pair_active(maps, dirs, m, d, acc_thres);
+            }
+        }
+    }
+    constexpr int WAVES = 16;
+    constexpr int PER_LANE = (P * WAVES + 63) / 64;
+    __shared__ int s_wcnt[P * WAVES];
     __shared__ int s_base;
-    const unsigned long long mask = __ballot(act);
     const int lane = threadIdx.x & 63, wv = threadIdx.x >> 6, nw = blockDim.x >> 6;
-    if (lane == 0) s_wcnt[wv] = __popcll(mask);
+    unsigned long long mask[P];
+#pragma unroll
+    for (int j = 0; j < P; ++j) {
+        mask[j] = __ballot(act[j]);
+        if (lane == 0) s_wcnt[j * nw + wv] = __popcll(mask[j]);
+    }
     __syncthreads();
-    if (threadIdx.x == 0) {
-        int tot = 0;
-        for (int q = 0; q < nw; ++q) { const int c = s_wcnt[q]; s_wcnt[q] = tot; tot += c; }
-        s_base = tot ? atomicAdd(n_active, tot) : 0;
+    if (wv == 0) {
+        const int cnts = P * nw;
+        int c[PER_LANE], sum = 0;
+#pragma unroll
+        for (int q = 0; q < PER_LANE; ++q) {
+            const int k = lane * PER_LANE + q;
+            c[q] = k < cnts ? s_wcnt[k] : 0;
+            sum += c[q];
+        }
+        int incl = sum;
+#pragma unroll
+        for (int dlt = 1; dlt < 64; dlt <<= 1) {
+            const int o = __shfl_up(incl, dlt, 64);
+            if (lane >= dlt) incl += o;
+        }
+        int run = incl - sum;
+#pragma unroll
+        for (int q = 0; q < PER_LANE; ++q) {
+            const int k = lane * PER_LANE + q;
+            if (k < cnts) s_wcnt[k] = run;
+            run += c[q];
+        }
+        if (lane == 63) s_base = incl ? atomicAdd(n_active, incl) : 0;
     }
     __syncthreads();
-    const int base = s_base + s_wcnt[wv];
-    if (act) {
-        const int64_t slot = (int64_t)base + __popcll(mask & ((1ull << lane) - 1ull));
-        if (slot < (int64_t)M * D) pair_ids[slot] = (int32_t)i;
-    } else if (in) {
-        if (vis) vis[i] = 0.0f;
-        if (rec_cnt) rec_cnt[i] = 0;
+#pragma unroll
+    for (int j = 0; j < P; ++j) {
+        if (act[j]) {
+            const int64_t slot = (int64_t)s_base + s_wcnt[j * nw + wv] + __popcll(mask[j] & ((1ull << lane) - 1ull));
+            if (slot < n) pair_ids[slot] = (int32_t)idx[j];
+        }
     }
 }
 
@@ -723,12 +778,14 @@
     if (M == 0) return TIR_OK;
     if (!maps || !rays || !dirs || !surf || !active) return TIR_ERR_ARG;
     int64_t n = (int64_t)M * D;
-    hipLaunchKernelGGL(k_shade_setup, dim3((unsigned)((n + 255) / 256)), dim3(256), 0, tir_stream(stream), maps,
+    hipLaunchKernelGGL(k_shade_setup<1>, dim3((unsigned)((n + 255) / 256)), dim3(256), 0, tir_stream(stream), maps,
                        rays, dirs, M, D, acc_thres, surf, active, (int32_t*)nullptr, (int32_t*)nullptr, (float*)nullptr,
                        (int32_t*)nullptr, 0);
     TIR_CHECK_LAUNCH();
     return TIR_OK;
 }
+
+extern "C" int tir_shade_setup_segment(void) { return 1024 * TIR_SETUP_PAIRS; }
 
 extern "C" int tir_shade_setup_compact(const float* maps, const float* rays, const float* dirs, int32_t M,
                                        int32_t D, float acc_thres, float* surf, uint8_t* active, int32_t* pair_ids,
@@ -740,8 +797,10 @@
     if (n >= ((int64_t)1 << 31)) return TIR_ERR_UNSUPPORTED;
     if (pair_order < 0 || pair_order > 2) return TIR_ERR_ARG;
     const int dir_major = pair_order == 2 ? 0 : 1;
-    hipLaunchKernelGGL(k_shade_setup, dim3((unsigned)((n + 1023) / 1024)), dim3(1024), 0, tir_stream(stream), maps,
-                       rays, dirs, M, D, acc_thres, surf, active, pair_ids, n_active, vis, ray_rec_cnt, dir_major);
+    constexpr int64_t per_block = 1024 * (int64_t)TIR_SETUP_PAIRS;
+    hipLaunchKernelGGL(k_shade_setup<TIR_SETUP_PAIRS>, dim3((unsigned)((n + per_block - 1) / per_block)), dim3(1024), 0,
+                       tir_stream(stream), maps, rays, dirs, M, D, acc_thres, surf, active, pair_ids, n_active, vis, ray_rec_cnt,
+                       dir_major);
     TIR_CHECK_LAUNCH();
     return TIR_OK;
 }
diff --git a/tensoir_amd/field_model.py b/tensoir_amd/field_model.py
--- a/tensoir_amd/field_model.py
+++ b/tensoir_amd/field_model.py
@@ -930,7 +930,7 @@
     def _step_words(self, dev):
         w = self.__dict__.get("_words")
         if w is None or w.device != torch.device(dev):
-            w = self.__dict__["_words"] = torch.zeros((8,), dtype=torch.int32, device=dev)
+            w = self.__dict__["_words"] = torch.zeros((ops.STEP_WORDS,), dtype=torch.int32, device=dev)
             self.__dict__["_pair_counter"] = w[0:1]
         return w
 
diff --git a/tensoir_amd/ops.py b/tensoir_amd/ops.py
--- a/tensoir_amd/ops.py
+++ b/tensoir_amd/ops.py
@@ -561,6 +561,15 @@
     return weight, acc, depth, tend, cnt
 
 
+STEP_TICKET_WORDS = 1056
+STEP_TICKET_OFFSET = 32
+STEP_WORDS = STEP_TICKET_OFFSET + STEP_TICKET_WORDS
+
+
+def _step_tickets(words):
+    return C.c_void_p(words.data_ptr() + 4 * STEP_TICKET_OFFSET) if words.numel() >= STEP_WORDS else None
+
+
 def march_primary_fused(field: TirField, rays, n_samples, t_stop, cap, words):
     rays = f32(rays, "rays", 6)
     B = rays.shape[0]
@@ -572,9 +581,11 @@
     off = torch.empty((B + 1,), dtype=torch.int32, device=dev)
     vd = torch.empty((B, 3), dtype=torch.float32, device=dev)
     total = words[5:6]
-    _call("tir_march_primary_fused_fwd", C.byref(field), _ptr(rays), None, B, n_samples, float(t_stop), _ptr(weight),
-          _ptr(acc), _ptr(depth), None, _ptr(cnt), _stats_ptr("tir_march_primary_fwd", dev), _ptr(vd),
-          C.c_void_p(words.data_ptr() + 4), 2, C.c_void_p(words.data_ptr() + 12), _ptr(off), int(cap), _ptr(total), _stream())
+    tickets = _step_tickets(words)
+    _call("tir_march_primary_fused_fwd" if tickets is None else "tir_march_primary_fused2_fwd", C.byref(field), _ptr(rays), None,
+          B, n_samples, float(t_stop), _ptr(weight), _ptr(acc), _ptr(depth), None, _ptr(cnt),
+          _stats_ptr("tir_march_primary_fwd", dev), _ptr(vd), C.c_void_p(words.data_ptr() + 4), 2,
+          C.c_void_p(words.data_ptr() + 12) if tickets is None else tickets, _ptr(off), int(cap), _ptr(total), _stream())
     return weight, acc, depth, cnt, off, total, vd
 
 
@@ -585,9 +596,11 @@
     out = torch.empty((B, MAP_STRIDE), dtype=torch.float32, device=rays.device)
     smooth = torch.zeros((2,), dtype=torch.float32, device=rays.device) if B == 0 else \
         torch.empty((2,), dtype=torch.float32, device=rays.device)
-    _call("tir_composite_primary_fused", _ptr(rays), _ptr(offsets), _ptr(rec_w), _ptr(rgb), _ptr(brdf), _ptr(brdf_jit),
-          _ptr(pred_n), _ptr(der_n), _ptr(acc), _ptr(depth), B, int(bool(white_bg)), int(bool(is_relight)),
-          float(fixed_fresnel), _ptr(out), C.c_void_p(words.data_ptr() + 16), _ptr(smooth), _ptr(rng_state), int(rng_step),
+    tickets = _step_tickets(words)
+    _call("tir_composite_primary_fused" if tickets is None else "tir_composite_primary_fused2", _ptr(rays), _ptr(offsets),
+          _ptr(rec_w), _ptr(rgb), _ptr(brdf), _ptr(brdf_jit), _ptr(pred_n), _ptr(der_n), _ptr(acc), _ptr(depth), B,
+          int(bool(white_bg)), int(bool(is_relight)), float(fixed_fresnel), _ptr(out),
+          C.c_void_p(words.data_ptr() + 16) if tickets is None else tickets, _ptr(smooth), _ptr(rng_state), int(rng_step),
           _stream())
     return out, smooth
 
```

New measurement: 4.968 million. About the same (-0.2%).
